# jinggqu/NextGen-UIA

Hardware: AMD Instinct MI355X
Metric: images/sec fwd+bwd BiomedCLIP+Mona bs=256 (higher is better)
Workload: dtype bf16

## Files before the change

include/uia_hip.h:

```cpp
#ifndef UIA_HIP_H
#define UIA_HIP_H
#include <stddef.h>
#include <stdint.h>

#ifdef __cplusplus
extern "C" {
#endif

enum { UIA_F32 = 0, UIA_BF16 = 1 };
enum { UIA_ACT_NONE = 0, UIA_ACT_GELU = 1, UIA_ACT_QUICKGELU = 2, UIA_ACT_RELU = 3 };
enum { UIA_MASK_NONE = 0, UIA_MASK_CAUSAL = 1, UIA_MASK_KEYPAD = 2 };
enum { UIA_MONA_BASELINE = 0, UIA_MONA_NOISE_AWARE = 1, UIA_MONA_FREQ_ENHANCED = 2, UIA_MONA_HYBRID = 3 };

const char* uia_last_error(void);
int uia_version(void);

typedef struct uia_gemm_desc {
    const void* A; int64_t lda;
    const void* W; int64_t ldw;
    int32_t M, N, K;
    float alpha;
    const float* bias;
    int32_t act;
    int32_t dact;
    const void* aux_in; int64_t ldaux_in;
    void* aux_out; int64_t ldaux_out;
    const float* resid; int64_t ldr;
    int32_t resid_mod, resid_row_off;
    const void* residT; int64_t ldrT;
    int32_t out_group;
    void* outT; int64_t ldo;
    float* out32; int64_t ldo32;
    int32_t w_kblocked;
    const void* resid_ln_stats;
    const float* resid_ln_w;
    const float* resid_ln_b;
    int64_t* rowsum_out;
    const int64_t* lnfold_sums;
    const float* lnfold_colsum;
    int32_t lnfold_dim; float lnfold_eps;
    int32_t resid_ln_dim; float resid_ln_eps;
    int64_t a_kb_rows;
    int64_t outT_kb_rows;
    int32_t* ln_flag;
    float ln_flag_limit;
    int32_t drop_where;
    float drop_p;
    uint64_t drop_seed;
    void* a_drop_out;
    float* splitk_ws;
    const void* A2;
    int64_t lda2;
    int32_t K2;
    int32_t a2_group_cols;
    int64_t a2_group_stride;
    const int8_t* resid_lo8;
    int64_t ld_resid_lo;
    int64_t residT_kb_rows;
    int8_t* out_lo8;
    int64_t ld_out_lo;
    int64_t resid_lo_kb_rows;
    int64_t out_lo_kb_rows;
} uia_gemm_desc;
int uia_gemm(void* stream, int dtype, const uia_gemm_desc* d, int tile_cfg );

int uia_wgrad(void* stream, int dtype, int M, int I, int J, const void* A, int64_t lda, const void* B, int64_t ldb,
              float alpha, float* dW, float* dbias_A);
int uia_wgrad_ex(void* stream, int dtype, int M, int I, int J, const void* A, int64_t lda, const void* B, int64_t ldb,
                 float alpha, float* dW, int64_t ldw, int i_valid, int j_valid, float* dbias_A);
int uia_wgrad_drop(void* stream, int dtype, int M, int I, int J, const void* A, int64_t lda, const void* B, int64_t ldb,
                   float alpha, float* dW, int64_t ldw, int i_valid, int j_valid, float drop_p, uint64_t seed, int64_t drop_ld, int drop_col0);
typedef struct uia_wgrad_group_desc {
    int32_t n, M, I, J;
    const void* A[4];
    const void* B[4];
    float* dW[4];
    float* dbias_A[4];
    int64_t lda, ldb, ldw;
    int32_t i_valid, j_valid;
    float alpha, drop_p;
    uint64_t drop_seed[4];
    int64_t drop_ld;
    int32_t drop_col0, reserved;
} uia_wgrad_group_desc;
int uia_wgrad_group(void* stream, int dtype, const uia_wgrad_group_desc* d);

typedef struct uia_attn_desc {
    const void *q, *k, *v; int64_t ld_qkv;
    void* out; int64_t ldo;
    float* lse;
    const int32_t* keylen;
    int32_t B, H, L, dh;
    int32_t mask_kind;
    float scale;
    const void* dout; int64_t lddo;
    void *dq, *dk, *dv; int64_t ld_dqkv;
    const int32_t* cu_seqlens;
    int64_t out_kb_rows;
    int64_t dqkv_kb_rows;
} uia_attn_desc;
int uia_attn_fwd(void* stream, int dtype, const uia_attn_desc* d);
int uia_attn_bwd(void* stream, int dtype, const uia_attn_desc* d);
int uia_attn_bwd_cfg(void* stream, int dtype, const uia_attn_desc* d, int cfg);

int uia_attn_fwd_long(void* stream, int dtype, const uia_attn_desc* d);

int uia_layernorm_fwd(void* stream, int dtype, int M, int D, int64_t ldx, const float* x, const float* gamma, const float* beta,
                      float eps, void* yT, float* y32);
int uia_layernorm_fwd_stats(void* stream, int dtype, int M, int D, int64_t ldx, const float* x, const float* gamma, const float* beta,
                            float eps, void* yT, float* y32, float* stats);
#define UIA_POOL_SLICES 32
int uia_ln_mean_rows(void* stream, int B, int L, int row0, int n, int D, int64_t ldx, const float* x, const float* gamma, const float* beta,
                     float eps, float* ws, float* out, int64_t ldo);
int uia_layernorm_bwd(void* stream, int dtype, int M, int D, int64_t ldx, const void* dy, const float* x, const float* gamma,
                      float eps, const float* dres, float* dx32, void* dxT);
int uia_layernorm_bwd3(void* stream, int dtype, int M, int D, int64_t ldx, const void* dy, const float* x, const void* x_hi, const int8_t* x_lo, int64_t x_kb_rows,
                       const float* gamma, float eps, const float* dres, const void* dres_hi, const int8_t* dres_lo, int64_t dres_kb_rows, float* dx32, void* dxT,
                       int8_t* dx_lo);

typedef struct uia_mona_spatial_desc {
    int32_t variant, B, h, w, bott;
    const void* t;
    void* d;
    const float *conv1_w, *conv1_b, *conv2_w, *conv2_b, *conv3_w, *conv3_b;
    const float *proj_w, *proj_b;
    const float* freq;
    const float *ne1_w, *ne1_b, *ne3_w, *ne3_b;
    float p_drop; uint64_t seed; const uint8_t* keep_mask;
    const void* dd;
    void* dt;
    float *g_conv1_w, *g_conv1_b, *g_conv2_w, *g_conv2_b, *g_conv3_w, *g_conv3_b, *g_proj_w, *g_proj_b, *g_freq,
          *g_ne1_w, *g_ne1_b, *g_ne3_w, *g_ne3_b;
    float* ws;
} uia_mona_spatial_desc;
size_t uia_mona_spatial_workspace_bytes(int B);
int uia_mona_pre_fwd(void* stream, int dtype, int M, int D, const float* x, const float* norm_w, const float* norm_b,
                     const float* gamma, const float* gammax, float eps, void* u);
int uia_mona_pre_fwd_t(void* stream, int dtype, int M, int D, const float* x, const float* norm_w, const float* norm_b, const float* gamma, const float* gammax,
                       float eps, void* u, const void* w1, int64_t ldw1, const float* b1, void* t, int64_t ldt);
int uia_mona_pre_bwd(void* stream, int dtype, int M, int D, const void* du, const float* x, const float* dy,
                     const float* norm_w, const float* norm_b, const float* gamma, const float* gammax, float eps,
                     float* dx32, void* dxT, float* g_gamma, float* g_gammax, float* g_norm_w, float* g_norm_b, float* ws,
                     int64_t dxT_kb_rows);
int uia_mona_pre_bwd_du(void* stream, int dtype, int M, int D, const void* dt, int64_t ldt, const void* w1t, int64_t ldw1, const float* x, const float* dy,
                        const float* norm_w, const float* norm_b, const float* gamma, const float* gammax, float eps,
                        float* dx32, void* dxT, float* g_gamma, float* g_gammax, float* g_norm_w, float* g_norm_b, float* ws, int64_t dxT_kb_rows);
int uia_mona_pre_bwd_du3(void* stream, int dtype, int M, int D, const void* dt, int64_t ldt, const void* w1t, int64_t ldw1, const float* x, const void* dy_hi, const int8_t* dy_lo,
                         const float* norm_w, const float* norm_b, const float* gamma, const float* gammax, float eps, void* dxT, int8_t* dx_lo, float* g_gamma,
                         float* g_gammax, float* g_norm_w, float* g_norm_b, float* ws, int64_t dxT_kb_rows);
size_t uia_mona_pre_bwd_workspace_bytes(int M, int D);
int uia_mona_spatial_fwd(void* stream, int dtype, const uia_mona_spatial_desc* d);
int uia_mona_spatial_bwd(void* stream, int dtype, const uia_mona_spatial_desc* d);

typedef struct uia_mona_fused_desc {
    uia_mona_spatial_desc sp;
    int32_t D; float eps;
    const float* x;
    const float *norm_w, *norm_b, *gamma, *gammax;
    const void* w1; const float* b1;
    const void* w2; const float* b2;
    float* y32;
    void* yT; int64_t yT_kb_rows;
    int64_t* rowsum_out;
    int32_t* ln_flag;
    void* u_out;
    void* t_out;
} uia_mona_fused_desc;
int uia_mona_fused_supported(int dtype, int D, int h, int w, int bott);
int uia_mona_fused_fwd(void* stream, int dtype, const uia_mona_fused_desc* d);

typedef struct uia_lora_rank_desc {
    int32_t M, N, nsrc;
    float alpha;
    const void* Q; int64_t ldq, q_stride;
    const void* W[3]; int64_t ldw;
    void* out; int64_t ldo;
    float drop_p;
    uint64_t seed[3];
} uia_lora_rank_desc;
int uia_lora_rank_update(void* stream, int dtype, const uia_lora_rank_desc* d);

typedef struct uia_ln_lora_desc {
    int32_t M, D, nsrc;
    float eps;
    const float* x; int64_t ldx;
    const float *gamma, *beta;
    void* h;
    const void* A[3]; int64_t lda;
    void* T; int64_t t_stride;
    float drop_p;
    uint64_t seed[3];
} uia_ln_lora_desc;
int uia_ln_lora_down(void* stream, int dtype, const uia_ln_lora_desc* d);

int uia_upsample_bilinear_fwd(void* stream, int B, int C, int h, int w, int H, int W, const float* src, int64_t ld, float* dst);
int uia_upsample_bilinear_bwd(void* stream, int B, int C, int h, int w, int H, int W, const float* ddst, float* dsrc, int64_t ld);
int uia_segment_mean_fwd(void* stream, int B, int n, int C, const float* x, int64_t ld, float* out);
int uia_segment_mean_bwd(void* stream, int B, int n, int C, const float* dout, float* dx, int64_t ld);
size_t uia_dicece_workspace_bytes(int B);
int uia_dicece_fwd_bwd(void* stream, int B, int C, int HW, const float* logits, const float* label, float smooth_nr, float smooth_dr,
                       float* ws, float* loss, float* dlogits);
size_t uia_focal_workspace_bytes(int N, int C);
int uia_focal_fwd_bwd(void* stream, int N, int C, const float* logits, const int64_t* labels, float gamma, float alpha, void* ws, size_t ws_bytes,
                      float* loss, float* dlogits);
size_t uia_binary_cls_stats_workspace_bytes(int N);
int uia_binary_cls_stats(void* stream, int N, const float* p1, const int64_t* labels, const int64_t* perm, void* ws, size_t ws_bytes, double* record);
size_t uia_surface_distances_workspace_bytes(int B, int H, int W);
int uia_surface_distances(void* stream, int B, int H, int W, const float* logits, const float* label, float percentile, void* ws, size_t ws_bytes,
                          double* hd, double* asd);

int uia_cast(void* stream, int dtype, size_t n, const float* src, void* dst, float scale);
int uia_transpose_cast(void* stream, int dtype, int rows, int cols, const float* src, void* dst);

typedef struct uia_pack_desc {
    const float* src;
    void* row;
    void* row_kb;
    void* tr;
    void* tr_kb;
    int32_t rows, cols;
    int32_t rows_pad, cols_pad;
    float scale;
    int32_t reserved_;
} uia_pack_desc;
int uia_pack_weights(void* stream, int dtype, int n, const uia_pack_desc* descs_device, int max_elems);
int uia_im2col(void* stream, int dtype, int B, int C, int H, int W, int P, const float* img, void* out);
int uia_im2col_padded(void* stream, int dtype, int B, int C, int H, int W, int P, const float* img, void* cols, int64_t ldo);
int uia_fill_cls(void* stream, int B, int N, int D, const float* cls, const float* pos0, float* x);
int uia_embed(void* stream, int rows, int L, int D, int vocab, int max_pos, const int64_t* ids, const float* table, const float* pos,
              const float* type0, float* out);
int uia_embed_packed(void* stream, int rows, int D, int vocab, int max_pos, const int64_t* ids, const int64_t* pos_idx, const float* table,
                     const float* pos, const float* type0, float* out);
int uia_embed_bwd(void* stream, int rows, int D, int vocab, const int64_t* ids, const float* dx, float* dtable, int64_t pad_id);
int uia_gather_rows(void* stream, int n, int D, const float* src, const int64_t* idx, float* dst);
int uia_dropout(void* stream, int dtype, size_t n, const void* src, void* dst, float p, uint64_t seed, int accumulate);
int uia_colsum(void* stream, int dtype, int M, int N, const void* A, int64_t lda, float* out);

int uia_layernorm_bwd_affine(void* stream, int dtype, int M, int D, const void* dy, const float* x, const float* gamma, float eps,
                             const float* dres, float* dx32, float* g_gamma, float* g_beta);
int uia_film_fwd(void* stream, int B, int N, int C, const float* x, const float* mul, const float* add, float* y);
int uia_film_bwd(void* stream, int B, int N, int C, const float* dy, const float* x, const float* mul, float* dx, float* dmul, float* dadd);
int uia_im2col3x3(void* stream, int dtype, int B, int h, int w, int C, int ntok, int tok_off, const float* x, void* cols);
int uia_col2im3x3(void* stream, int dtype, int B, int h, int w, int C, int ntok, int tok_off, const void* dcols, float* dx);
int uia_unshuffle(void* stream, int dtype, int B, int h, int w, int k1, int k2, const void* tmp, int64_t ld, float bias, float* out);
int uia_shuffle(void* stream, int dtype, int B, int h, int w, int k1, int k2, const float* dout, void* dtmp, int64_t ld);
int uia_act_bwd(void* stream, int dtype, size_t n, const void* dy, const void* y, int act, void* out);

size_t uia_infonce_workspace_bytes(int B, int E);
int uia_infonce_fwd_bwd(void* stream, int B, int E, const float* img, const float* txt, float inv_temp, float grad_scale,
                        float* loss, float* dimg, float* dtxt, void* workspace, size_t workspace_bytes);

int uia_adamw_clip_step(void* stream, size_t n, float* p, const float* g, float* m, float* v, float lr, float beta1, float beta2,
                        float eps, float weight_decay, float max_norm, int step, float grad_scale, float* ws2);

int uia_grad_accum_guarded(void* stream, size_t n, float* acc, float* mb, const float* loss, float* stats, int32_t* ctl, uint8_t* ok_log, int64_t log_index);
int uia_adamw_clip_step_guarded(void* stream, size_t n, float* p, float* acc, float* m, float* v, float lr, float lr_min, int t_max, float beta1, float beta2,
                                float eps, float weight_decay, float max_norm, float grad_scale, float skip_scale, float* ws8, int32_t* ctl);

enum { UIA_CONV3 = 0, UIA_CONVT_FWD = 1, UIA_CONVT_BWD = 2, UIA_CONV1 = 3 };
#define UIA_WGRAD_MAX_SPLITS 64
#define UIA_WGRAD_MAX_NARROW_SPLITS 512
#define UIA_WGRAD_MAX_DIRECT_SPLITS 1024
int uia_conv_igemm(void* stream, int dtype, int mode, int B, int H, int W, int C1, int C2, const void* x1, const void* x2, int N, int N1,
                   const void* w, const float* bias, void* y1, void* y2);
int uia_conv_wgrad_splits(int mode, int B, int H, int W, int C1, int C2, int N);
int uia_conv_igemm_form(int mode, int C1, int C2, int N, int N1);
int uia_conv_wgrad_form(int mode, int C1, int C2, int N);
int uia_conv_wgrad(void* stream, int dtype, int mode, int B, int H, int W, int C1, int C2, const void* x1, const void* x2, int N, const void* dy,
                   float* ws, float* dw);
#define UIA_BN_SLICES 256
int uia_bn_fwd(void* stream, int dtype, int training, int64_t M, int C, const void* y, const float* gamma, const float* beta, float* running_mean,
               float* running_var, int64_t* num_batches_tracked, float momentum, float eps, float* ws, float* mean, float* invstd, float* scale,
               float* shift, int relu, void* out);
int uia_bn_relu_bwd(void* stream, int dtype, int64_t M, int C, const void* y, const void* dout, const float* scale, const float* shift,
                    const float* mean, const float* invstd, const float* gamma, float* ws, float* dgamma, float* dbeta, void* dy);
int uia_colsum_ordered(void* stream, int dtype, int64_t M, int C, const void* y, float* ws, float* out);
int uia_bn_act_fwd(void* stream, int dtype, int training, int64_t M, int C, const void* y, const float* gamma, const float* beta, float* running_mean,
                   float* running_var, int64_t* num_batches_tracked, float momentum, float eps, float* ws, float* mean, float* invstd, float* scale,
                   float* shift, float slope, void* out, float drop_p, uint64_t seed, const uint8_t* keep_mask);
int uia_bn_act_bwd(void* stream, int dtype, int64_t M, int C, const void* y, const void* dout, const float* scale, const float* shift,
                   const float* mean, const float* invstd, const float* gamma, float* ws, float* dgamma, float* dbeta, void* dy, float slope,
                   float drop_p, uint64_t seed, const uint8_t* keep_mask);
int uia_maxpool2_fwd(void* stream, int dtype, int B, int H, int W, int C, const void* x, void* y);
int uia_maxpool2_bwd(void* stream, int dtype, int B, int H, int W, int C, const void* x, const void* dy, void* dx);
int uia_upsample_ac(void* stream, int dtype, int backward, int B, int H, int W, int C, int f, const void* in, void* out);
int uia_resize_aa(void* stream, int dtype, int backward, int B, int C, int Hi, int Wi, int Ho, int Wo, const void* x, float* tmp, float* out,
                  const float* dout, void* dx);

int uia_conv_strided(void* stream, int dtype, int dgrad, int B, int H, int W, int C, int k, int s, const void* x, int N, const void* w, void* y);
int uia_conv_strided_wgrad_splits(int B, int H, int W, int C, int k, int s, int N);
int uia_conv_strided_form(int dgrad, int C, int N, int k, int s);
int uia_conv_strided_wgrad_form(int C, int N, int k, int s);
int uia_conv_strided_wgrad(void* stream, int dtype, int B, int H, int W, int C, int k, int s, const void* x, int N, const void* dy, float* ws,
                           float* dw);
int uia_maxpool3s2_fwd(void* stream, int dtype, int B, int H, int W, int C, const void* x, void* y);
int uia_maxpool3s2_bwd(void* stream, int dtype, int B, int H, int W, int C, const void* x, const void* dy, void* dx);
int uia_bn_add_relu_fwd(void* stream, int dtype, int training, int64_t M, int C, const void* y, const void* r, const float* gamma, const float* beta,
                        float* running_mean, float* running_var, int64_t* num_batches_tracked, float momentum, float eps, float* ws, float* mean,
                        float* invstd, float* scale, float* shift, void* out);
int uia_bn_add_relu_bwd(void* stream, int dtype, int64_t M, int C, const void* y, const void* out, const void* dout, const float* mean,
                        const float* invstd, const float* gamma, float* ws, float* dgamma, float* dbeta, void* dy, void* dr);
int uia_avgpool_fwd(void* stream, int dtype, int B, int H, int W, int C, const void* x, float* pooled);
int uia_avgpool_bwd(void* stream, int dtype, int B, int H, int W, int C, const float* dout, void* dx);
int uia_nchw_to_nhwc(void* stream, int dtype, int B, int Cin, int H, int W, int Cout, int rep, const float* x, void* out);
int uia_add2(void* stream, int dtype, int64_t n, const void* a, const void* b, void* out);

int uia_comm_unique_id_bytes(void);
int uia_comm_get_unique_id(void* out, int bytes);
int uia_comm_init(int rank, int world, const void* unique_id, int bytes);
int uia_comm_world(void);
int uia_comm_initialised(void);
int uia_allreduce_sum(void* stream, int dtype, void* buf, size_t n);
int uia_allgather(void* stream, int dtype, const void* send, void* recv, size_t n_per_rank);
int uia_comm_destroy(void);

#ifdef __cplusplus
}
// ... 3 lines not shown
```

nextgen-uia_amd/csrc/capi.cpp:

```cpp
#include "uia_kernels.h"

void uia_set_error(const char* fmt, ...);
#define NEED(ptr, name) do { if (!(ptr)) { uia_set_error("%s: null descriptor", name); return -1; } } while (0)

extern "C" {

int uia_version(void) { return 100; }

int uia_gemm(void* stream, int dtype, const uia_gemm_desc* d, int tile_cfg) {
    NEED(d, "uia_gemm");
    return uia_gemm_launch((hipStream_t)stream, dtype, *d, tile_cfg);
}
int uia_lora_rank_update(void* stream, int dtype, const uia_lora_rank_desc* d) {
    NEED(d, "uia_lora_rank_update");
    return uia_lora_rank_update_launch((hipStream_t)stream, dtype, *d);
}
int uia_ln_lora_down(void* stream, int dtype, const uia_ln_lora_desc* d) {
    NEED(d, "uia_ln_lora_down");
    return uia_ln_lora_down_launch((hipStream_t)stream, dtype, *d);
}
int uia_wgrad(void* stream, int dtype, int M, int I, int J, const void* A, int64_t lda, const void* B, int64_t ldb, float alpha, float* dW, float* dbias_A) {
    return uia_wgrad_launch((hipStream_t)stream, dtype, M, I, J, A, lda, B, ldb, alpha, dW, dbias_A);
}
int uia_wgrad_ex(void* stream, int dtype, int M, int I, int J, const void* A, int64_t lda, const void* B, int64_t ldb, float alpha, float* dW, int64_t ldw,
                 int i_valid, int j_valid, float* dbias_A) {
    if (ldw <= 0) { uia_set_error("uia_wgrad_ex: ldw=%lld must be positive", (long long)ldw); return -1; }
    return uia_wgrad_launch((hipStream_t)stream, dtype, M, I, J, A, lda, B, ldb, alpha, dW, dbias_A, ldw, i_valid, j_valid);
}
int uia_wgrad_group(void* stream, int dtype, const uia_wgrad_group_desc* d) {
    if (!d) { uia_set_error("uia_wgrad_group: null descriptor"); return -1; }
    if (d->n < 1 || d->n > 4) { uia_set_error("uia_wgrad_group: n=%d outside 1..4", d->n); return -1; }
    if (d->ldw <= 0) { uia_set_error("uia_wgrad_group: ldw=%lld must be positive", (long long)d->ldw); return -1; }
    float* dW[4];
    float* db[4];
    for (int g = 0; g < 4; ++g) { dW[g] = d->dW[g]; db[g] = d->dbias_A[g]; }
    if (d->drop_p > 0.f) for (int g = 0; g < d->n; ++g) if (db[g]) { uia_set_error("uia_wgrad_group: dbias with dropout on B is not a form of the kernel"); return -1; }
    return uia_wgrad_group_launch((hipStream_t)stream, dtype, d->n, d->M, d->I, d->J, d->A, (long)d->lda, d->B, (long)d->ldb, d->alpha, dW, db, (long)d->ldw, d->i_valid, d->j_valid,
                                  d->drop_p, d->drop_seed, (long)d->drop_ld, d->drop_col0);
}
int uia_wgrad_drop(void* stream, int dtype, int M, int I, int J, const void* A, int64_t lda, const void* B, int64_t ldb, float alpha, float* dW, int64_t ldw,
                   int i_valid, int j_valid, float drop_p, uint64_t seed, int64_t drop_ld, int drop_col0) {
    if (ldw <= 0) { uia_set_error("uia_wgrad_drop: ldw=%lld must be positive", (long long)ldw); return -1; }
    if (!(drop_p > 0.f)) { uia_set_error("uia_wgrad_drop: drop_p=%f must be in (0, 1); uia_wgrad_ex is the form without dropout", (double)drop_p); return -1; }
    return uia_wgrad_launch((hipStream_t)stream, dtype, M, I, J, A, lda, B, ldb, alpha, dW, nullptr, ldw, i_valid, j_valid, drop_p, seed, drop_ld, drop_col0);
}
int uia_attn_fwd(void* stream, int dtype, const uia_attn_desc* d) {
    NEED(d, "uia_attn_fwd");
    return uia_attn_fwd_launch((hipStream_t)stream, dtype, *d);
}
int uia_attn_fwd_long(void* stream, int dtype, const uia_attn_desc* d) {
    NEED(d, "uia_attn_fwd_long");
    return uia_attn_fwd_long_launch((hipStream_t)stream, dtype, *d);
}
int uia_attn_bwd(void* stream, int dtype, const uia_attn_desc* d) {
    NEED(d, "uia_attn_bwd");
    return uia_attn_bwd_launch((hipStream_t)stream, dtype, *d, 0);
}
int uia_attn_bwd_cfg(void* stream, int dtype, const uia_attn_desc* d, int cfg) {
    NEED(d, "uia_attn_bwd_cfg");
    return uia_attn_bwd_launch((hipStream_t)stream, dtype, *d, cfg);
}
int uia_layernorm_fwd(void* stream, int dtype, int M, int D, int64_t ldx, const float* x, const float* gamma, const float* beta, float eps, void* yT, float* y32) {
    return uia_layernorm_fwd_launch((hipStream_t)stream, dtype, M, D, ldx, x, gamma, beta, eps, yT, y32, nullptr);
}
int uia_layernorm_fwd_stats(void* stream, int dtype, int M, int D, int64_t ldx, const float* x, const float* gamma, const float* beta, float eps, void* yT, float* y32,
                            float* stats) {
    return uia_layernorm_fwd_launch((hipStream_t)stream, dtype, M, D, ldx, x, gamma, beta, eps, yT, y32, stats);
}
int uia_layernorm_bwd(void* stream, int dtype, int M, int D, int64_t ldx, const void* dy, const float* x, const float* gamma, float eps, const float* dres, float* dx32, void* dxT) {
    return uia_layernorm_bwd_launch((hipStream_t)stream, dtype, M, D, ldx, dy, x, gamma, eps, dres, dx32, dxT);
}
int uia_layernorm_bwd3(void* stream, int dtype, int M, int D, int64_t ldx, const void* dy, const float* x, const void* x_hi, const int8_t* x_lo, int64_t x_kb_rows,
                       const float* gamma, float eps, const float* dres, const void* dres_hi, const int8_t* dres_lo, int64_t dres_kb_rows, float* dx32, void* dxT,
                       int8_t* dx_lo) {
    return uia_layernorm_bwd3_launch((hipStream_t)stream, dtype, M, D, ldx, dy, x, x_hi, x_lo, (long)x_kb_rows, gamma, eps, dres, dres_hi, dres_lo, (long)dres_kb_rows, dx32, dxT,
                                     dx_lo);
}
int uia_cast(void* stream, int dtype, size_t n, const float* src, void* dst, float scale) { return uia_cast_launch((hipStream_t)stream, dtype, n, src, dst, scale); }
int uia_transpose_cast(void* stream, int dtype, int rows, int cols, const float* src, void* dst) { return uia_transpose_cast_launch((hipStream_t)stream, dtype, rows, cols, src, dst); }
int uia_pack_weights(void* stream, int dtype, int n, const uia_pack_desc* descs_device, int max_elems) { return uia_pack_weights_launch((hipStream_t)stream, dtype, n, descs_device, max_elems); }
int uia_im2col(void* stream, int dtype, int B, int C, int H, int W, int P, const float* img, void* out) { return uia_im2col_launch((hipStream_t)stream, dtype, B, C, H, W, P, img, out); }
int uia_fill_cls(void* stream, int B, int N, int D, const float* cls, const float* pos0, float* x) { return uia_fill_cls_launch((hipStream_t)stream, B, N, D, cls, pos0, x); }
int uia_embed(void* stream, int rows, int L, int D, int vocab, int max_pos, const int64_t* ids, const float* table, const float* pos, const float* type0, float* out) {
    return uia_embed_launch((hipStream_t)stream, rows, L, D, vocab, max_pos, ids, table, pos, type0, out);
}
int uia_gather_rows(void* stream, int n, int D, const float* src, const int64_t* idx, float* dst) { return uia_gather_rows_launch((hipStream_t)stream, n, D, src, idx, dst); }

int uia_mona_pre_fwd(void* stream, int dtype, int M, int D, const float* x, const float* norm_w, const float* norm_b, const float* gamma,
                     const float* gammax, float eps, void* u) {
    return uia_mona_pre_fwd_launch((hipStream_t)stream, dtype, M, D, x, norm_w, norm_b, gamma, gammax, eps, u);
}
int uia_mona_pre_bwd(void* stream, int dtype, int M, int D, const void* du, const float* x, const float* dy, const float* norm_w,
                     const float* norm_b, const float* gamma, const float* gammax, float eps, float* dx32, void* dxT, float* g_gamma,
                     float* g_gammax, float* g_norm_w, float* g_norm_b, float* ws, int64_t dxT_kb_rows) {
    return uia_mona_pre_bwd_launch((hipStream_t)stream, dtype, M, D, du, x, dy, norm_w, norm_b, gamma, gammax, eps, dx32, dxT, g_gamma, g_gammax,
                                   g_norm_w, g_norm_b, ws, (long)dxT_kb_rows);
}
int uia_mona_pre_fwd_t(void* stream, int dtype, int M, int D, const float* x, const float* norm_w, const float* norm_b, const float* gamma, const float* gammax,
                       float eps, void* u, const void* w1, int64_t ldw1, const float* b1, void* t, int64_t ldt) {
    return uia_mona_pre_fwd_t_launch((hipStream_t)stream, dtype, M, D, x, norm_w, norm_b, gamma, gammax, eps, u, w1, (long)ldw1, b1, t, (long)ldt);
}
int uia_mona_pre_bwd_du(void* stream, int dtype, int M, int D, const void* dt, int64_t ldt, const void* w1t, int64_t ldw1, const float* x, const float* dy,
                        const float* norm_w, const float* norm_b, const float* gamma, const float* gammax, float eps, float* dx32, void* dxT, float* g_gamma,
                        float* g_gammax, float* g_norm_w, float* g_norm_b, float* ws, int64_t dxT_kb_rows) {
    if (!dt || !w1t) { uia_set_error("uia_mona_pre_bwd_du: null dt / w1t"); return -1; }
    return uia_mona_pre_bwd_launch((hipStream_t)stream, dtype, M, D, nullptr, x, dy, norm_w, norm_b, gamma, gammax, eps, dx32, dxT, g_gamma, g_gammax,
                                   g_norm_w, g_norm_b, ws, (long)dxT_kb_rows, dt, (long)ldt, w1t, (long)ldw1);
}
int uia_mona_pre_bwd_du3(void* stream, int dtype, int M, int D, const void* dt, int64_t ldt, const void* w1t, int64_t ldw1, const float* x, const void* dy_hi, const int8_t* dy_lo,
                         const float* norm_w, const float* norm_b, const float* gamma, const float* gammax, float eps, void* dxT, int8_t* dx_lo, float* g_gamma,
                         float* g_gammax, float* g_norm_w, float* g_norm_b, float* ws, int64_t dxT_kb_rows) {
    if (!dt || !w1t || !dy_hi || !dy_lo || !dx_lo) { uia_set_error("uia_mona_pre_bwd_du3: null dt / w1t / dy_hi / dy_lo / dx_lo"); return -1; }
    return uia_mona_pre_bwd_launch((hipStream_t)stream, dtype, M, D, nullptr, x, nullptr, norm_w, norm_b, gamma, gammax, eps, nullptr, dxT, g_gamma, g_gammax,
                                   g_norm_w, g_norm_b, ws, (long)dxT_kb_rows, dt, (long)ldt, w1t, (long)ldw1, dy_hi, dy_lo, dx_lo);
}
size_t uia_mona_pre_bwd_workspace_bytes(int M, int D) { return uia_mona_pre_bwd_ws_floats(M, D) * sizeof(float); }
int uia_mona_spatial_fwd(void* stream, int dtype, const uia_mona_spatial_desc* d) {
    NEED(d, "uia_mona_spatial_fwd");
    return uia_mona_spatial_fwd_launch((hipStream_t)stream, dtype, *d);
}
int uia_mona_spatial_bwd(void* stream, int dtype, const uia_mona_spatial_desc* d) {
    NEED(d, "uia_mona_spatial_bwd");
    return uia_mona_spatial_bwd_launch((hipStream_t)stream, dtype, *d);
}
int uia_mona_fused_fwd(void* stream, int dtype, const uia_mona_fused_desc* d) {
    NEED(d, "uia_mona_fused_fwd");
    return uia_mona_fused_fwd_launch((hipStream_t)stream, dtype, *d);
}

size_t uia_infonce_workspace_bytes(int B, int E) { return uia_infonce_workspace_floats(B, E) * sizeof(float); }
int uia_infonce_fwd_bwd(void* stream, int B, int E, const float* img, const float* txt, float inv_temp, float grad_scale, float* loss,
                        float* dimg, float* dtxt, void* workspace, size_t workspace_bytes) {
    return uia_infonce_launch((hipStream_t)stream, B, E, img, txt, inv_temp, grad_scale, loss, dimg, dtxt, (float*)workspace, workspace_bytes / sizeof(float));
}
int uia_adamw_clip_step(void* stream, size_t n, float* p, const float* g, float* m, float* v, float lr, float beta1, float beta2, float eps,
                        float weight_decay, float max_norm, int step, float grad_scale, float* ws2) {
    return uia_adamw_clip_launch((hipStream_t)stream, n, p, g, m, v, lr, beta1, beta2, eps, weight_decay, max_norm, step, grad_scale, ws2);
}
int uia_grad_accum_guarded(void* stream, size_t n, float* acc, float* mb, const float* loss, float* stats, int32_t* ctl, uint8_t* ok_log, int64_t log_index) {
    return uia_grad_accum_guarded_launch((hipStream_t)stream, n, acc, mb, loss, stats, (int*)ctl, ok_log, (long)log_index);
}
int uia_adamw_clip_step_guarded(void* stream, size_t n, float* p, float* acc, float* m, float* v, float lr, float lr_min, int t_max, float beta1, float beta2,
                                float eps, float weight_decay, float max_norm, float grad_scale, float skip_scale, float* ws8, int32_t* ctl) {
    return uia_adamw_clip_guarded_launch((hipStream_t)stream, n, p, acc, m, v, lr, lr_min, t_max, beta1, beta2, eps, weight_decay, max_norm, grad_scale, skip_scale, ws8, (int*)ctl);
}

int uia_dropout(void* stream, int dtype, size_t n, const void* src, void* dst, float p, uint64_t seed, int accumulate) {
    return uia_dropout_launch((hipStream_t)stream, dtype, n, src, dst, p, seed, accumulate);
}
int uia_colsum(void* stream, int dtype, int M, int N, const void* A, int64_t lda, float* out) {
    return uia_colsum_launch((hipStream_t)stream, dtype, M, N, A, lda, out);
}

int uia_layernorm_bwd_affine(void* stream, int dtype, int M, int D, const void* dy, const float* x, const float* gamma, float eps, const float* dres,
                             float* dx32, float* g_gamma, float* g_beta) {
    return uia_layernorm_bwd_affine_launch((hipStream_t)stream, dtype, M, D, dy, x, gamma, eps, dres, dx32, g_gamma, g_beta);
}
int uia_film_fwd(void* stream, int B, int N, int C, const float* x, const float* mul, const float* add, float* y) { return uia_film_fwd_launch((hipStream_t)stream, B, N, C, x, mul, add, y); }
int uia_film_bwd(void* stream, int B, int N, int C, const float* dy, const float* x, const float* mul, float* dx, float* dmul, float* dadd) {
    return uia_film_bwd_launch((hipStream_t)stream, B, N, C, dy, x, mul, dx, dmul, dadd);
// ... 155 lines not shown
```

nextgen-uia_amd/csrc/layernorm.hip:

```cpp
#include "uia_common.h"
#include "uia_kernels.h"

namespace {

constexpr int LN_MAXV = 4;

template <typename T>
__global__ __launch_bounds__(256) void ln_fwd_kernel(int M, int D, long ldx, const float* __restrict__ x, const float* __restrict__ gamma,
                                                      const float* __restrict__ beta, float eps, T* __restrict__ yT, float* __restrict__ y32,
                                                      float* __restrict__ stats) {
    const int row = blockIdx.x * 4 + (threadIdx.x >> 6), lane = threadIdx.x & 63;
    if (row >= M) return;
    const int nv = D >> 2;
    const float* xr = x + (size_t)row * ldx;
    f32x4 v[LN_MAXV];
    float s = 0.f;
#pragma unroll
    for (int k = 0; k < LN_MAXV; ++k) {
        const int c = lane + 64 * k;
        v[k] = c < nv ? load4(xr + 4 * c) : f32x4{0.f, 0.f, 0.f, 0.f};
        s += v[k][0] + v[k][1] + v[k][2] + v[k][3];
    }
    const float mean = wave_sum(s) / D;
    float q = 0.f;
#pragma unroll
    for (int k = 0; k < LN_MAXV; ++k) {
        const int c = lane + 64 * k;
        if (c < nv) {
#pragma unroll
            for (int e = 0; e < 4; ++e) { const float d = v[k][e] - mean; q = fmaf(d, d, q); }
        }
    }
    const float rstd = rsqrtf(wave_sum(q) / D + eps);
    if (stats && lane == 0) *(float2*)(stats + 2 * (size_t)row) = float2{mean, rstd};
#pragma unroll
    for (int k = 0; k < LN_MAXV; ++k) {
        const int c = lane + 64 * k;
        if (c < nv) {
            const f32x4 g = load4(gamma + 4 * c), b = load4(beta + 4 * c);
            f32x4 y;
#pragma unroll
            for (int e = 0; e < 4; ++e) y[e] = fmaf((v[k][e] - mean) * rstd, g[e], b[e]);
            if (yT) store4(yT + (size_t)row * D + 4 * c, y);
            if (y32) store4(y32 + (size_t)row * D + 4 * c, y);
        }
    }
}

template <typename T, bool THREE, int NV>
__global__ __launch_bounds__(256, NV == 4 ? (THREE ? 3 : 5) : 1) void ln_bwd_kernel(int M, int D, long ldx, const T* __restrict__ dy, const float* __restrict__ x,
                                                      const float* __restrict__ gamma, float eps, const float* __restrict__ dres,
                                                      float* __restrict__ dx32, T* __restrict__ dxT,
                                                      const bf16_t* __restrict__ x_hi, const int8_t* __restrict__ x_lo, long x_kb_rows,
                                                      const bf16_t* __restrict__ dres_hi, const int8_t* __restrict__ dres_lo, long dres_kb_rows, int8_t* __restrict__ dx_lo) {
    const int row = blockIdx.x * 4 + (threadIdx.x >> 6), lane = threadIdx.x & 63;
    if (row >= M) return;
    const int nv = D >> 2;
    const float* xr = x + (size_t)row * ldx;
    const T* dyr = dy + (size_t)row * D;
    f32x4 v[NV], g[NV];
    uint2 rhi[THREE ? NV : 1];
    unsigned rlo[THREE ? NV : 1];
    const bool r3 = THREE && dres_lo != nullptr;
    float s = 0.f;
#pragma unroll
    for (int k = 0; k < NV; ++k) {
        const int c = lane + 64 * k;
        v[k] = f32x4{0.f, 0.f, 0.f, 0.f};
        g[k] = f32x4{0.f, 0.f, 0.f, 0.f};
        if constexpr (THREE) { rhi[k] = uint2{0u, 0u}; rlo[k] = 0u; }
        if (c < nv) {
            if (THREE && x_lo) {
                const bf16_t* hp = x_kb_rows ? x_hi + ((size_t)((4 * c) >> 5) * (size_t)x_kb_rows + row) * 32 + ((4 * c) & 31) : x_hi + (size_t)row * D + 4 * c;
                v[k] = three_byte_load4(hp, x_lo + (size_t)row * D + 4 * c);
            } else {
                v[k] = load4(xr + 4 * c);
            }
            const f32x4 d = load4(dyr + 4 * c), w = load4(gamma + 4 * c);
            if constexpr (THREE) {
                if (r3) {
                    rhi[k] = *(const uint2*)(dres_kb_rows ? dres_hi + ((size_t)((4 * c) >> 5) * (size_t)dres_kb_rows + row) * 32 + ((4 * c) & 31) : dres_hi + (size_t)row * D + 4 * c);
                    rlo[k] = *(const unsigned*)(dres_lo + (size_t)row * D + 4 * c);
                }
            }
#pragma unroll
            for (int e = 0; e < 4; ++e) g[k][e] = d[e] * w[e];
        }
        s += v[k][0] + v[k][1] + v[k][2] + v[k][3];
    }
    const float mean = wave_sum(s) / D;
    float q = 0.f;
#pragma unroll
    for (int k = 0; k < NV; ++k) {
        const int c = lane + 64 * k;
#pragma unroll
        for (int e = 0; e < 4; ++e) {
            const float d = c < nv ? v[k][e] - mean : 0.f;
            v[k][e] = d;
            q = fmaf(d, d, q);
        }
    }
    const float rstd = rsqrtf(wave_sum(q) / D + eps);
    float sg = 0.f, sgx = 0.f;
#pragma unroll
    for (int k = 0; k < NV; ++k)
#pragma unroll
        for (int e = 0; e < 4; ++e) {
            v[k][e] *= rstd;
            sg += g[k][e];
            sgx = fmaf(g[k][e], v[k][e], sgx);
        }
    const float mg = wave_sum(sg) / D, mgx = wave_sum(sgx) / D;
#pragma unroll
    for (int k = 0; k < NV; ++k) {
        const int c = lane + 64 * k;
        if (c < nv) {
            f32x4 o = f32x4{0.f, 0.f, 0.f, 0.f};
            if constexpr (THREE) {
                if (r3) o = three_byte_decode4(rhi[k], rlo[k]);
                else if (dres) o = load4(dres + (size_t)row * ldx + 4 * c);
            } else {
                if (dres) o = load4(dres + (size_t)row * ldx + 4 * c);
            }
#pragma unroll
            for (int e = 0; e < 4; ++e) o[e] += rstd * (g[k][e] - mg - v[k][e] * mgx);
            if (dx32) store4(dx32 + (size_t)row * ldx + 4 * c, o);
            if constexpr (sizeof(T) == 2) {
                if (THREE && dx_lo) three_byte_store4((bf16_t*)dxT + (size_t)row * D + 4 * c, dx_lo + (size_t)row * D + 4 * c, o);
                else if (dxT) store4(dxT + (size_t)row * ldx + 4 * c, o);
            } else {
                if (dxT) store4(dxT + (size_t)row * ldx + 4 * c, o);
            }
        }
    }
}

}

int uia_layernorm_fwd_launch(hipStream_t stream, int dtype, int M, int D, long ldx, const float* x, const float* gamma, const float* beta,
                             float eps, void* yT, float* y32, float* stats) {
    UIA_CHECK_ARG(M > 0 && D > 0 && D % 4 == 0 && D <= 1024, "uia_layernorm_fwd: unsupported shape M=%d D=%d", M, D);
    UIA_CHECK_ARG(x && gamma && beta && (yT || y32 || stats), "uia_layernorm_fwd: null tensor");
    UIA_CHECK_ARG(ldx >= D && ldx % 4 == 0, "uia_layernorm_fwd: row stride %ld", ldx);
    UIA_CHECK_ARG(((uintptr_t)x | (uintptr_t)gamma | (uintptr_t)beta | (uintptr_t)yT | (uintptr_t)y32 | (uintptr_t)stats) % 8 == 0, "uia_layernorm_fwd: alignment");
    const dim3 grid((M + 3) / 4), block(256);
    if (dtype == UIA_BF16) hipLaunchKernelGGL(ln_fwd_kernel<bf16_t>, grid, block, 0, stream, M, D, ldx, x, gamma, beta, eps, (bf16_t*)yT, y32, stats);
    else if (dtype == UIA_F32) hipLaunchKernelGGL(ln_fwd_kernel<float>, grid, block, 0, stream, M, D, ldx, x, gamma, beta, eps, (float*)yT, y32, stats);
    else { uia_set_error("uia_layernorm_fwd: bad dtype %d", dtype); return -1; }
    UIA_CHECK_LAUNCH();
    return 0;
}

int uia_layernorm_bwd_launch(hipStream_t stream, int dtype, int M, int D, long ldx, const void* dy, const float* x, const float* gamma, float eps,
                             const float* dres, float* dx32, void* dxT) {
    return uia_layernorm_bwd3_launch(stream, dtype, M, D, ldx, dy, x, nullptr, nullptr, 0, gamma, eps, dres, nullptr, nullptr, 0, dx32, dxT, nullptr);
}

int uia_layernorm_bwd3_launch(hipStream_t stream, int dtype, int M, int D, long ldx, const void* dy, const float* x, const void* x_hi, const int8_t* x_lo,
                              long x_kb_rows, const float* gamma, float eps, const float* dres, const void* dres_hi, const int8_t* dres_lo, long dres_kb_rows,
                              float* dx32, void* dxT, int8_t* dx_lo) {
    UIA_CHECK_ARG(M > 0 && D > 0 && D % 4 == 0 && D <= 1024, "uia_layernorm_bwd: unsupported shape M=%d D=%d", M, D);
    UIA_CHECK_ARG(dy && (x || (x_hi && x_lo)) && gamma && (dx32 || dxT), "uia_layernorm_bwd: null tensor");
    UIA_CHECK_ARG(ldx >= D && ldx % 4 == 0, "uia_layernorm_bwd: row stride %ld", ldx);
    const bool three = x_lo || dres_lo || dx_lo;
    UIA_CHECK_ARG(!three || (dtype == UIA_BF16 && ldx == D), "uia_layernorm_bwd: three-byte tensors need bf16 and compact rows (ldx == D)");
    UIA_CHECK_ARG(!x_lo || (x_hi && !x && (x_kb_rows == 0 || (x_kb_rows >= M && D % 32 == 0)) && ((uintptr_t)x_hi % 8) == 0 && ((uintptr_t)x_lo % 4) == 0),
                  "uia_layernorm_bwd: x as a three-byte tensor needs x_hi + x_lo (and no fp32 x), a K-blocked hi plane of at least M rows and D a multiple of 32");
    UIA_CHECK_ARG(!dres_lo || (dres_hi && !dres && ((uintptr_t)dres_hi % 8) == 0 && ((uintptr_t)dres_lo % 4) == 0), "uia_layernorm_bwd: dres as a three-byte tensor needs dres_hi + dres_lo (and no fp32 dres)");
    UIA_CHECK_ARG(!dx_lo || (dxT && ((uintptr_t)dxT % 8) == 0 && ((uintptr_t)dx_lo % 4) == 0), "uia_layernorm_bwd: dx_lo needs dxT as the hi plane");
    UIA_CHECK_ARG(x_lo || x_kb_rows == 0, "uia_layernorm_bwd: x_kb_rows without a three-byte x");
    UIA_CHECK_ARG(dres_kb_rows == 0 || (dres_lo && dres_kb_rows >= M && D % 32 == 0), "uia_layernorm_bwd: dres_kb_rows needs a three-byte dres, at least M rows per column block and D a multiple of 32");
    const dim3 grid((M + 3) / 4), block(256);
#define UIA_LN_BWD(TT, TH, NVV)                                                                                                              \
    hipLaunchKernelGGL((ln_bwd_kernel<TT, TH, NVV>), grid, block, 0, stream, M, D, ldx, (const TT*)dy, x, gamma, eps, dres, dx32, (TT*)dxT,          \
                       (const bf16_t*)x_hi, x_lo, x_kb_rows, (const bf16_t*)dres_hi, dres_lo, dres_kb_rows, dx_lo)
    const bool narrow = D <= 768;
    if (dtype == UIA_BF16 && three) { if (narrow) UIA_LN_BWD(bf16_t, true, 3); else UIA_LN_BWD(bf16_t, true, 4); }
    else if (dtype == UIA_BF16) { if (narrow) UIA_LN_BWD(bf16_t, false, 3); else UIA_LN_BWD(bf16_t, false, 4); }
    else if (dtype == UIA_F32) { if (narrow) UIA_LN_BWD(float, false, 3); else UIA_LN_BWD(float, false, 4); }
#undef UIA_LN_BWD
    else { uia_set_error("uia_layernorm_bwd: bad dtype %d", dtype); return -1; }
    UIA_CHECK_LAUNCH();
    return 0;
}
```

nextgen-uia_amd/csrc/uia_kernels.h:

```cpp
#pragma once
#include <hip/hip_runtime.h>
#include <stddef.h>
#include <stdint.h>

#include "../../include/uia_hip.h"

typedef uia_gemm_desc UiaGemmParams;
typedef uia_attn_desc UiaAttnParams;

int uia_gemm_launch(hipStream_t stream, int dtype, const UiaGemmParams& p, int cfg);
int uia_attn_fwd_launch(hipStream_t stream, int dtype, const UiaAttnParams& p);
int uia_attn_fwd_long_launch(hipStream_t stream, int dtype, const UiaAttnParams& p);
int uia_attn_bwd_launch(hipStream_t stream, int dtype, const UiaAttnParams& p, int cfg = 0);
int uia_layernorm_fwd_launch(hipStream_t stream, int dtype, int M, int D, long ldx, const float* x, const float* gamma, const float* beta,
                             float eps, void* yT, float* y32, float* stats);
int uia_layernorm_bwd_launch(hipStream_t stream, int dtype, int M, int D, long ldx, const void* dy, const float* x, const float* gamma, float eps,
                             const float* dres, float* dx32, void* dxT);
int uia_layernorm_bwd3_launch(hipStream_t stream, int dtype, int M, int D, long ldx, const void* dy, const float* x, const void* x_hi, const int8_t* x_lo,
                              long x_kb_rows, const float* gamma, float eps, const float* dres, const void* dres_hi, const int8_t* dres_lo, long dres_kb_rows,
                              float* dx32, void* dxT, int8_t* dx_lo);
int uia_lora_rank_update_launch(hipStream_t stream, int dtype, const uia_lora_rank_desc& p);
int uia_ln_lora_down_launch(hipStream_t stream, int dtype, const uia_ln_lora_desc& p);
int uia_cast_launch(hipStream_t stream, int dtype, size_t n, const float* src, void* dst, float scale);
int uia_transpose_cast_launch(hipStream_t stream, int dtype, int rows, int cols, const float* src, void* dst);
int uia_pack_weights_launch(hipStream_t stream, int dtype, int n, const uia_pack_desc* descs_device, int max_elems);
int uia_im2col_launch(hipStream_t stream, int dtype, int B, int C, int H, int W, int P, const float* img, void* out);
int uia_fill_cls_launch(hipStream_t stream, int B, int N, int D, const float* cls, const float* pos0, float* x);
int uia_embed_launch(hipStream_t stream, int rows, int L, int D, int vocab, int max_pos, const int64_t* ids, const float* table, const float* pos, const float* type0, float* out);
int uia_gather_rows_launch(hipStream_t stream, int n, int D, const float* src, const int64_t* idx, float* dst);
int uia_wgrad_group_launch(hipStream_t stream, int dtype, int n, int M, int I, int J, const void* const* A, long lda, const void* const* B, long ldb, float alpha,
                            float* const* dW, float* const* dbias, long ldw, int i_valid, int j_valid, float drop_p, const uint64_t* drop_seed, long drop_ld, int drop_col0);
int uia_wgrad_launch(hipStream_t stream, int dtype, int M, int I, int J, const void* A, long lda, const void* B, long ldb, float alpha, float* dW, float* dbias,
                     long ldw = 0, int i_valid = 0, int j_valid = 0, float drop_p = 0.f, uint64_t drop_seed = 0, long drop_ld = 0, int drop_col0 = 0);
int uia_mona_pre_fwd_launch(hipStream_t stream, int dtype, int M, int D, const float* x, const float* nw, const float* nb, const float* gamma,
                            const float* gammax, float eps, void* u);
int uia_mona_pre_fwd_t_launch(hipStream_t stream, int dtype, int M, int D, const float* x, const float* nw, const float* nb, const float* gamma,
                              const float* gammax, float eps, void* u, const void* w1, long ldw1, const float* b1, void* t, long ldt);
int uia_mona_pre_bwd_launch(hipStream_t stream, int dtype, int M, int D, const void* du, const float* x, const float* dy, const float* nw,
                            const float* nb, const float* gamma, const float* gammax, float eps, float* dx32, void* dxT, float* g_gamma,
                            float* g_gammax, float* g_nw, float* g_nb, float* ws, long dxT_kb_rows, const void* dt = nullptr, long ldt = 0,
                            const void* w1t = nullptr, long ldw1 = 0, const void* dy_hi = nullptr, const int8_t* dy_lo = nullptr, int8_t* dx_lo = nullptr);
size_t uia_mona_pre_bwd_ws_floats(int M, int D);
int uia_mona_spatial_fwd_launch(hipStream_t stream, int dtype, const uia_mona_spatial_desc& p);
int uia_mona_spatial_bwd_launch(hipStream_t stream, int dtype, const uia_mona_spatial_desc& p);
int uia_mona_fused_fwd_launch(hipStream_t stream, int dtype, const uia_mona_fused_desc& q);
size_t uia_infonce_workspace_floats(int B, int E);
int uia_infonce_launch(hipStream_t stream, int B, int E, const float* img, const float* txt, float inv_temp, float grad_scale, float* loss,
                       float* dimg, float* dtxt, float* ws, size_t ws_floats);
int uia_adamw_clip_launch(hipStream_t stream, size_t n, float* p, const float* g, float* m, float* v, float lr, float beta1, float beta2,
                          float eps, float weight_decay, float max_norm, int step, float grad_scale, float* ws);
int uia_grad_accum_guarded_launch(hipStream_t stream, size_t n, float* acc, float* mb, const float* loss, float* stats, int* ctl, unsigned char* ok_log, long log_index);
int uia_adamw_clip_guarded_launch(hipStream_t stream, size_t n, float* p, float* acc, float* m, float* v, float lr, float lr_min, int t_max, float beta1,
                                  float beta2, float eps, float weight_decay, float max_norm, float grad_scale, float skip_scale, float* ws8, int* ctl);
int uia_dropout_launch(hipStream_t stream, int dtype, size_t n, const void* src, void* dst, float p, uint64_t seed, int accumulate);
int uia_colsum_launch(hipStream_t stream, int dtype, int M, int N, const void* A, long lda, float* out);
int uia_attn_small_launch(hipStream_t stream, int dtype, const UiaAttnParams& p, bool bwd);
bool uia_attn_dh16_ok(int dtype, const UiaAttnParams& p);
int uia_attn_dh16_launch(hipStream_t stream, const UiaAttnParams& p, bool bwd);
int uia_layernorm_bwd_affine_launch(hipStream_t stream, int dtype, int M, int D, const void* dy, const float* x, const float* gamma, float eps,
                                    const float* dres, float* dx32, float* g_gamma, float* g_beta);
int uia_film_fwd_launch(hipStream_t stream, int B, int N, int C, const float* x, const float* mul, const float* add, float* y);
int uia_film_bwd_launch(hipStream_t stream, int B, int N, int C, const float* dy, const float* x, const float* mul, float* dx, float* dmul, float* dadd);
int uia_im2col3x3_launch(hipStream_t stream, int dtype, int B, int h, int w, int C, int ntok, int tok_off, const float* x, void* cols);
int uia_col2im3x3_launch(hipStream_t stream, int dtype, int B, int h, int w, int C, int ntok, int tok_off, const void* dcols, float* dx);
int uia_unshuffle_launch(hipStream_t stream, int dtype, int B, int h, int w, int k1, int k2, const void* tmp, long ld, float bias, float* out);
int uia_shuffle_launch(hipStream_t stream, int dtype, int B, int h, int w, int k1, int k2, const float* dout, void* dtmp, long ld);
int uia_act_bwd_launch(hipStream_t stream, int dtype, size_t n, const void* dy, const void* y, int act, void* out);
size_t uia_mona_spatial_ws_floats(int B);
int uia_upsample_bilinear_launch(hipStream_t stream, bool bwd, int B, int C, int h, int w, int H, int W, const float* in, float* out, long ld);
int uia_segment_mean_launch(hipStream_t stream, bool bwd, int B, int n, int C, const float* in, float* out, long ld);
size_t uia_dicece_ws_floats(int B);
int uia_dicece_launch(hipStream_t stream, int B, int C, int HW, const float* logits, const float* label, float nr, float dr, float* ws, float* loss, float* dlogits);
size_t uia_focal_ws_bytes(int N, int C);
int uia_focal_launch(hipStream_t stream, int N, int C, const float* logits, const int64_t* labels, float gamma, float alpha, void* ws, size_t ws_bytes,
                     float* loss, float* dlogits);
size_t uia_binary_cls_stats_ws_bytes(int N);
int uia_binary_cls_stats_launch(hipStream_t stream, int N, const float* p1, const int64_t* labels, const int64_t* perm, void* ws, size_t ws_bytes,
                                double* record);
size_t uia_surface_ws_bytes(int B, int H, int W);
int uia_surface_launch(hipStream_t stream, int B, int H, int W, const float* logits, const float* label, float percentile, void* ws, size_t ws_bytes,
                       double* hd, double* asd);
int uia_im2col_padded_launch(hipStream_t stream, int dtype, int B, int C, int H, int W, int P, const float* img, void* out, long ldo);
int uia_embed_bwd_launch(hipStream_t stream, int rows, int D, int vocab, const int64_t* ids, const float* dx, float* dtable, long pad_id);
int uia_embed_packed_launch(hipStream_t stream, int rows, int D, int vocab, int max_pos, const int64_t* ids, const int64_t* pos_idx, const float* table, const float* pos, const float* type0, float* out);
int uia_ln_mean_rows_launch(hipStream_t stream, int B, int L, int row0, int n, int D, long ldx, const float* x, const float* gamma, const float* beta,
                            float eps, float* ws, float* out, long ldo);
int uia_conv_igemm_launch(hipStream_t stream, int dtype, int mode, int B, int H, int W, int C1, int C2, const void* x1, const void* x2, int N, int N1,
                          const void* w, const float* bias, void* y1, void* y2);
int uia_conv_wgrad_splits(int mode, int B, int H, int W, int C1, int C2, int N);
int uia_conv_wgrad_launch(hipStream_t stream, int dtype, int mode, int B, int H, int W, int C1, int C2, const void* x1, const void* x2, int N,
                          const void* dy, float* ws, float* dw);
int uia_bn_fwd_launch(hipStream_t stream, int dtype, int training, long M, int C, const void* y, const float* gamma, const float* beta,
                      float* run_mean, float* run_var, int64_t* nbt, float momentum, float eps, float* ws, float* mean, float* invstd,
                      float* scale, float* shift, int relu, void* out);
int uia_bn_relu_bwd_launch(hipStream_t stream, int dtype, long M, int C, const void* y, const void* dout, const float* scale, const float* shift,
                           const float* mean, const float* invstd, const float* gamma, float* ws, float* dgamma, float* dbeta, void* dy);
int uia_colsum_ordered_launch(hipStream_t stream, int dtype, long M, int C, const void* y, float* ws, float* out);
int uia_conv_igemm_form(int mode, int C1, int C2, int N, int N1);
int uia_conv_wgrad_form(int mode, int C1, int C2, int N);
int uia_bn_act_fwd_launch(hipStream_t stream, int dtype, int training, long M, int C, const void* y, const float* gamma, const float* beta,
                          float* run_mean, float* run_var, int64_t* nbt, float momentum, float eps, float* ws, float* mean, float* invstd,
                          float* scale, float* shift, float slope, void* out, float drop_p, uint64_t seed, const uint8_t* keep_mask);
int uia_bn_act_bwd_launch(hipStream_t stream, int dtype, long M, int C, const void* y, const void* dout, const float* scale, const float* shift,
// ... 23 lines not shown
```

nextgen-uia_amd/uia_hip/_lib.py:

```python
import ctypes as C
import os
import re

import torch

_HERE = os.path.dirname(os.path.abspath(__file__))
LIB_PATH = os.environ.get("UIA_HIP_LIB") or os.path.join(_HERE, "libuia_hip.so")

F32, BF16 = 0, 1
ACT_NONE, ACT_GELU, ACT_QUICKGELU, ACT_RELU = 0, 1, 2, 3
MASK_NONE, MASK_CAUSAL, MASK_KEYPAD = 0, 1, 2
MONA_VARIANTS = {"baseline": 0, "noise_aware": 1, "freq_enhanced": 2, "hybrid": 3}

vp, i32, i64, f32, sz = C.c_void_p, C.c_int32, C.c_int64, C.c_float, C.c_size_t


class PackDesc(C.Structure):
    _fields_ = [("src", vp), ("row", vp), ("row_kb", vp), ("tr", vp), ("tr_kb", vp), ("rows", i32), ("cols", i32),
                ("rows_pad", i32), ("cols_pad", i32), ("scale", f32), ("reserved_", i32)]


class GemmDesc(C.Structure):
    _fields_ = [("A", vp), ("lda", i64), ("W", vp), ("ldw", i64), ("M", i32), ("N", i32), ("K", i32), ("alpha", f32),
                ("bias", vp), ("act", i32), ("dact", i32), ("aux_in", vp), ("ldaux_in", i64), ("aux_out", vp), ("ldaux_out", i64),
# ... 70 lines not shown
    "uia_conv_wgrad_form": (C.c_int, [C.c_int, C.c_int, C.c_int, C.c_int]),
    "uia_bn_act_fwd": (C.c_int, [vp, C.c_int, C.c_int, i64, C.c_int, vp, vp, vp, vp, vp, vp, f32, f32, vp, vp, vp, vp, vp, f32, vp, f32, C.c_uint64, vp]),
    "uia_bn_act_bwd": (C.c_int, [vp, C.c_int, i64, C.c_int, vp, vp, vp, vp, vp, vp, vp, vp, vp, vp, vp, f32, f32, C.c_uint64, vp]),
    "uia_maxpool2_fwd": (C.c_int, [vp, C.c_int, C.c_int, C.c_int, C.c_int, C.c_int, vp, vp]),
    "uia_maxpool2_bwd": (C.c_int, [vp, C.c_int, C.c_int, C.c_int, C.c_int, C.c_int, vp, vp, vp]),
    "uia_conv_strided": (C.c_int, [vp, C.c_int, C.c_int, C.c_int, C.c_int, C.c_int, C.c_int, C.c_int, C.c_int, vp, C.c_int, vp, vp]),
    "uia_conv_strided_wgrad_splits": (C.c_int, [C.c_int, C.c_int, C.c_int, C.c_int, C.c_int, C.c_int, C.c_int]),
    "uia_conv_strided_form": (C.c_int, [C.c_int, C.c_int, C.c_int, C.c_int, C.c_int]),
    "uia_conv_strided_wgrad_form": (C.c_int, [C.c_int, C.c_int, C.c_int, C.c_int]),
    "uia_conv_strided_wgrad": (C.c_int, [vp, C.c_int, C.c_int, C.c_int, C.c_int, C.c_int, C.c_int, C.c_int, vp, C.c_int, vp, vp, vp]),
    "uia_maxpool3s2_fwd": (C.c_int, [vp, C.c_int, C.c_int, C.c_int, C.c_int, C.c_int, vp, vp]),
    "uia_maxpool3s2_bwd": (C.c_int, [vp, C.c_int, C.c_int, C.c_int, C.c_int, C.c_int, vp, vp, vp]),
    "uia_bn_add_relu_fwd": (C.c_int, [vp, C.c_int, C.c_int, i64, C.c_int, vp, vp, vp, vp, vp, vp, vp, f32, f32, vp, vp, vp, vp, vp, vp]),
    "uia_bn_add_relu_bwd": (C.c_int, [vp, C.c_int, i64, C.c_int, vp, vp, vp, vp, vp, vp, vp, vp, vp, vp, vp]),
    "uia_avgpool_fwd": (C.c_int, [vp, C.c_int, C.c_int, C.c_int, C.c_int, C.c_int, vp, vp]),
    "uia_avgpool_bwd": (C.c_int, [vp, C.c_int, C.c_int, C.c_int, C.c_int, C.c_int, vp, vp]),
    "uia_nchw_to_nhwc": (C.c_int, [vp, C.c_int, C.c_int, C.c_int, C.c_int, C.c_int, C.c_int, C.c_int, vp, vp]),
    "uia_add2": (C.c_int, [vp, C.c_int, i64, vp, vp, vp]),
    "uia_bn_fwd": (C.c_int, [vp, C.c_int, C.c_int, i64, C.c_int, vp, vp, vp, vp, vp, vp, f32, f32, vp, vp, vp, vp, vp, C.c_int, vp]),
    "uia_bn_relu_bwd": (C.c_int, [vp, C.c_int, i64, C.c_int, vp, vp, vp, vp, vp, vp, vp, vp, vp, vp, vp]),
    "uia_colsum_ordered": (C.c_int, [vp, C.c_int, i64, C.c_int, vp, vp, vp]),
    "uia_upsample_ac": (C.c_int, [vp, C.c_int, C.c_int, C.c_int, C.c_int, C.c_int, C.c_int, C.c_int, vp, vp]),
    "uia_resize_aa": (C.c_int, [vp, C.c_int, C.c_int, C.c_int, C.c_int, C.c_int, C.c_int, C.c_int, C.c_int, vp, vp, vp, vp, vp]),
    "uia_layernorm_bwd": (C.c_int, [vp, C.c_int, C.c_int, C.c_int, i64, vp, vp, vp, f32, vp, vp, vp]),
    "uia_ln_lora_down": (C.c_int, [vp, C.c_int, C.POINTER(LnLoraDesc)]),
    "uia_lora_rank_update": (C.c_int, [vp, C.c_int, C.POINTER(LoraRankDesc)]),
    "uia_layernorm_bwd3": (C.c_int, [vp, C.c_int, C.c_int, C.c_int, i64, vp, vp, vp, vp, i64, vp, f32, vp, vp, vp, i64, vp, vp, vp]),
    "uia_mona_pre_fwd": (C.c_int, [vp, C.c_int, C.c_int, C.c_int, vp, vp, vp, vp, vp, f32, vp]),
    "uia_mona_pre_bwd": (C.c_int, [vp, C.c_int, C.c_int, C.c_int, vp, vp, vp, vp, vp, vp, vp, f32, vp, vp, vp, vp, vp, vp, vp, i64]),
    "uia_mona_pre_fwd_t": (C.c_int, [vp, C.c_int, C.c_int, C.c_int, vp, vp, vp, vp, vp, f32, vp, vp, i64, vp, vp, i64]),
    "uia_mona_pre_bwd_du": (C.c_int, [vp, C.c_int, C.c_int, C.c_int, vp, i64, vp, i64, vp, vp, vp, vp, vp, vp, f32, vp, vp, vp, vp, vp, vp, vp, i64]),
    "uia_mona_pre_bwd_du3": (C.c_int, [vp, C.c_int, C.c_int, C.c_int, vp, i64, vp, i64, vp, vp, vp, vp, vp, vp, vp, f32, vp, vp, vp, vp, vp, vp, vp, i64]),
    "uia_mona_pre_bwd_workspace_bytes": (sz, [C.c_int, C.c_int]),
    "uia_mona_spatial_fwd": (C.c_int, [vp, C.c_int, C.POINTER(MonaSpatialDesc)]),
    "uia_mona_spatial_bwd": (C.c_int, [vp, C.c_int, C.POINTER(MonaSpatialDesc)]),
    "uia_mona_spatial_workspace_bytes": (sz, [C.c_int]),
    "uia_mona_fused_supported": (C.c_int, [C.c_int, C.c_int, C.c_int, C.c_int, C.c_int]),
    "uia_mona_fused_fwd": (C.c_int, [vp, C.c_int, C.POINTER(MonaFusedDesc)]),
    "uia_upsample_bilinear_fwd": (C.c_int, [vp, C.c_int, C.c_int, C.c_int, C.c_int, C.c_int, C.c_int, vp, C.c_int64, vp]),
    "uia_upsample_bilinear_bwd": (C.c_int, [vp, C.c_int, C.c_int, C.c_int, C.c_int, C.c_int, C.c_int, vp, vp, C.c_int64]),
    "uia_segment_mean_fwd": (C.c_int, [vp, C.c_int, C.c_int, C.c_int, vp, C.c_int64, vp]),
    "uia_segment_mean_bwd": (C.c_int, [vp, C.c_int, C.c_int, C.c_int, vp, vp, C.c_int64]),
    "uia_dicece_workspace_bytes": (sz, [C.c_int]),
    "uia_dicece_fwd_bwd": (C.c_int, [vp, C.c_int, C.c_int, C.c_int, vp, vp, C.c_float, C.c_float, vp, vp, vp]),
    "uia_focal_workspace_bytes": (sz, [C.c_int, C.c_int]),
    "uia_focal_fwd_bwd": (C.c_int, [vp, C.c_int, C.c_int, vp, vp, f32, f32, vp, sz, vp, vp]),
    "uia_binary_cls_stats_workspace_bytes": (sz, [C.c_int]),
    "uia_binary_cls_stats": (C.c_int, [vp, C.c_int, vp, vp, vp, vp, sz, vp]),
    "uia_surface_distances_workspace_bytes": (sz, [C.c_int, C.c_int, C.c_int]),
    "uia_surface_distances": (C.c_int, [vp, C.c_int, C.c_int, C.c_int, vp, vp, f32, vp, sz, vp, vp]),
    "uia_infonce_workspace_bytes": (sz, [C.c_int, C.c_int]),
    "uia_infonce_fwd_bwd": (C.c_int, [vp, C.c_int, C.c_int, vp, vp, f32, f32, vp, vp, vp, vp, sz]),
    "uia_adamw_clip_step": (C.c_int, [vp, sz, vp, vp, vp, vp, f32, f32, f32, f32, f32, f32, C.c_int, f32, vp]),
    "uia_grad_accum_guarded": (C.c_int, [vp, sz, vp, vp, vp, vp, vp, vp, i64]),
    "uia_adamw_clip_step_guarded": (C.c_int, [vp, sz, vp, vp, vp, vp, f32, f32, C.c_int, f32, f32, f32, f32, f32, f32, f32, vp, vp]),
    "uia_comm_unique_id_bytes": (C.c_int, []),
    "uia_comm_get_unique_id": (C.c_int, [vp, C.c_int]),
    "uia_comm_init": (C.c_int, [C.c_int, C.c_int, vp, C.c_int]),
    "uia_comm_world": (C.c_int, []),
    "uia_comm_initialised": (C.c_int, []),
    "uia_allreduce_sum": (C.c_int, [vp, C.c_int, vp, sz]),
    "uia_allgather": (C.c_int, [vp, C.c_int, vp, vp, sz]),
    "uia_comm_destroy": (C.c_int, []),
    "uia_dropout": (C.c_int, [vp, C.c_int, sz, vp, vp, f32, C.c_uint64, C.c_int]),
    "uia_colsum": (C.c_int, [vp, C.c_int, C.c_int, C.c_int, vp, i64, vp]),
    "uia_layernorm_bwd_affine": (C.c_int, [vp, C.c_int, C.c_int, C.c_int, vp, vp, vp, f32, vp, vp, vp, vp]),
    "uia_film_fwd": (C.c_int, [vp, C.c_int, C.c_int, C.c_int, vp, vp, vp, vp]),
    "uia_film_bwd": (C.c_int, [vp, C.c_int, C.c_int, C.c_int, vp, vp, vp, vp, vp, vp]),
    "uia_im2col3x3": (C.c_int, [vp, C.c_int, C.c_int, C.c_int, C.c_int, C.c_int, C.c_int, C.c_int, vp, vp]),
    "uia_col2im3x3": (C.c_int, [vp, C.c_int, C.c_int, C.c_int, C.c_int, C.c_int, C.c_int, C.c_int, vp, vp]),
    "uia_unshuffle": (C.c_int, [vp, C.c_int, C.c_int, C.c_int, C.c_int, C.c_int, C.c_int, vp, i64, f32, vp]),
    "uia_shuffle": (C.c_int, [vp, C.c_int, C.c_int, C.c_int, C.c_int, C.c_int, C.c_int, vp, vp, i64]),
    "uia_act_bwd": (C.c_int, [vp, C.c_int, sz, vp, vp, C.c_int, vp]),
    "uia_cast": (C.c_int, [vp, C.c_int, sz, vp, vp, f32]),
    "uia_transpose_cast": (C.c_int, [vp, C.c_int, C.c_int, C.c_int, vp, vp]),
    "uia_pack_weights": (C.c_int, [vp, C.c_int, C.c_int, vp, C.c_int]),
    "uia_im2col": (C.c_int, [vp, C.c_int, C.c_int, C.c_int, C.c_int, C.c_int, C.c_int, vp, vp]),
    "uia_im2col_padded": (C.c_int, [vp, C.c_int, C.c_int, C.c_int, C.c_int, C.c_int, C.c_int, vp, vp, C.c_int64]),
    "uia_fill_cls": (C.c_int, [vp, C.c_int, C.c_int, C.c_int, vp, vp, vp]),
    "uia_embed": (C.c_int, [vp, C.c_int, C.c_int, C.c_int, C.c_int, C.c_int, vp, vp, vp, vp, vp]),
    "uia_embed_bwd": (C.c_int, [vp, C.c_int, C.c_int, C.c_int, vp, vp, vp, C.c_int64]),
    "uia_embed_packed": (C.c_int, [vp, C.c_int, C.c_int, C.c_int, C.c_int, vp, vp, vp, vp, vp, vp]),
    "uia_gather_rows": (C.c_int, [vp, C.c_int, C.c_int, vp, vp, vp]),
}

_lib = None
_BLOCKING = ("uia_comm_init", "uia_comm_destroy", "uia_comm_get_unique_id")


class UiaError(RuntimeError):
    pass


def lib():
    global _lib
    if _lib is None:
        if not os.path.exists(LIB_PATH):
            raise UiaError(f"{LIB_PATH} not built: run `make -C nextgen-uia_amd/csrc` (hipcc --offload-arch=gfx950). "
                           "There is no CPU fallback for the uia hot path.")
        release = os.environ.get("UIA_CTYPES_RELEASE_GIL", "0") == "1"
        handle = (C.CDLL if release else C.PyDLL)(LIB_PATH)
        blocking = C.CDLL(LIB_PATH)
        _one_copy_of("librccl")
        _one_copy_of("libamdhip64")
        for name, (res, args) in PROTOTYPES.items():
            fn = getattr(blocking if name in _BLOCKING else handle, name)
            fn.restype, fn.argtypes = res, args
            if name in _BLOCKING:
                setattr(handle, name, fn)
        _lib = handle
    return _lib


def _one_copy_of(stem):
    try:
        pat = re.compile(r"^" + re.escape(stem) + r"\.so(\.\d+)*$")
        paths = {line.split()[-1] for line in open("/proc/self/maps") if pat.match(os.path.basename(line.split()[-1]) if line.split() else "")}
    except OSError:
        return
    real = {os.path.realpath(p) for p in paths}
    if len(real) > 1:
        raise UiaError(f"two copies of {stem} are loaded ({sorted(real)}): import torch before uia_hip so that libuia_hip.so binds to PyTorch's runtime")


def check(rc, what=""):
    if rc != 0:
        raise UiaError(f"{what} failed (rc={rc}): {lib().uia_last_error().decode()}")
```

nextgen-uia_amd/uia_hip/functional.py:

```python
import math
import os
import weakref

import time

import torch

from . import handoff, ops
from ._lib import UiaError
from .handoff import (Resid3, _g3_partner_feeds, fwd3_of, grad3_decode, grad3_of, grad_resid3_enabled, hook_free, linear_chain,
                      publish_fwd3, publish_grad3, publish_rows, publish_t_copy, set_grad_resid3, t_copy_of, take_rows, zero_sums)
from .handoff import clear as clear_t_copies

_STATE = {"dtype": torch.bfloat16, "seed": 0x5EED, "calls": 0, "fwd_resid3": os.environ.get("UIA_FWD_RESID3", "1") != "0"}


def set_compute_dtype(dt):
    assert dt in (torch.bfloat16, torch.float32)
    _STATE["dtype"] = dt


def compute_dtype():
    return _STATE["dtype"]


def set_deferred_text_ln(flag):
    _STATE["text_ln_deferred"] = bool(flag)


def set_block_resid3(flag):
    _STATE["block_resid3"] = bool(flag)


def set_fwd_resid3(flag):
    _STATE["fwd_resid3"] = bool(flag)


def set_text_resid3(flag):
    _STATE["text_resid3"] = bool(flag)


def set_ln_fold(flag):
    _STATE["ln_fold"] = bool(flag)


def set_deterministic(flag):
    _STATE["deterministic"] = bool(flag)
    ops.TAIL_SPLIT_K = not flag


def ln_fold_enabled(dt, rows=None):
    return dt != torch.float32 and _STATE.get("ln_fold", True) and (rows is None or rows > _STATE.get("ln_fold_min_rows", 2048))


class LnFoldRangeError(FloatingPointError):
    """A GEMM that left row sums for a folded LayerNorm saw a non-finite or out-of-range partial sum: the LayerNorm statistics of that
    row — and everything downstream of it — are wrong."""


_FOLD_POLL = {}
_FOLD_REPORTED = {}


POLL_LAG = max(1, int(os.environ.get("UIA_POLL_LAG", "2")))


def reset_ln_flag(device=None):
    dev = torch.device("cuda", torch.cuda.current_device()) if device is None else torch.device(device)
    key = dev.index if dev.index is not None else torch.cuda.current_device()
    _FOLD_POLL.pop(key, None)
    _FOLD_REPORTED.pop(key, None)
    if key in ops._LN_FLAG:
        ops._LN_FLAG[key].zero_()


def poll_ln_flag(device=None, sync=False):
    dev = torch.device("cuda", torch.cuda.current_device()) if device is None else torch.device(device)
    key = dev.index if dev.index is not None else torch.cuda.current_device()
    flag = ops._LN_FLAG.get(key)
    if flag is None:
        return 0
    seen = 0
    pending = _FOLD_POLL.setdefault(key, [])
    while pending and (sync or len(pending) >= POLL_LAG):
        prev = pending.pop(0)
        t0 = time.perf_counter()
        prev[1].synchronize()
        _STATE["gpu_wait_s"] = _STATE.get("gpu_wait_s", 0.0) + time.perf_counter() - t0
        seen |= int(prev[0][0])
    host = torch.empty(1, dtype=torch.int32, pin_memory=True)
    host.copy_(flag, non_blocking=True)
    ev = torch.cuda.Event()
    ev.record()
    if sync:
# ... 234 lines not shown


def _act(M, K, dt, like, n_consumer):
    if ops.kb_ok(M, n_consumer, K, dt):
        return ops.kb_empty(M, K, dt, like.device)
    return torch.empty((M, K), device=like.device, dtype=dt)


def _attn_act(M, K, dt, like, n_consumer):
    return _act(M, K, dt, like, n_consumer) if dt == torch.bfloat16 else torch.empty((M, K), device=like.device, dtype=dt)


def _as_act(buf, M, K, dt, n_consumer):
    if ops.kb_ok(M, n_consumer, K, dt):
        return buf if ops.is_kb(buf) else ops.KBlocked.over(buf.view(M, K))
    return buf.as_rows() if ops.is_kb(buf) else buf


MONA_PARAM_ORDER = ("gamma", "gammax", "project1.weight", "project1.bias", "project2.weight", "project2.bias", "norm.weight", "norm.bias",
                    "adapter_conv.conv1.weight", "adapter_conv.conv1.bias", "adapter_conv.conv2.weight", "adapter_conv.conv2.bias",
                    "adapter_conv.conv3.weight", "adapter_conv.conv3.bias", "adapter_conv.projector.weight", "adapter_conv.projector.bias",
                    "adapter_conv.freq_filter", "adapter_conv.noise_estimator.1.weight", "adapter_conv.noise_estimator.1.bias",
                    "adapter_conv.noise_estimator.3.weight", "adapter_conv.noise_estimator.3.bias")
_SPATIAL_MAP = {"adapter_conv.conv1.weight": "conv1_w", "adapter_conv.conv1.bias": "conv1_b", "adapter_conv.conv2.weight": "conv2_w",
                "adapter_conv.conv2.bias": "conv2_b", "adapter_conv.conv3.weight": "conv3_w", "adapter_conv.conv3.bias": "conv3_b",
                "adapter_conv.projector.weight": "proj_w", "adapter_conv.projector.bias": "proj_b", "adapter_conv.freq_filter": "freq",
                "adapter_conv.noise_estimator.1.weight": "ne1_w", "adapter_conv.noise_estimator.1.bias": "ne1_b",
                "adapter_conv.noise_estimator.3.weight": "ne3_w", "adapter_conv.noise_estimator.3.bias": "ne3_b"}


class MonaFn(torch.autograd.Function):

    @staticmethod
    def forward(ctx, x, variant, hw, p_drop, keep_mask, names, direct, *params):
        P = dict(zip(names, params))
        B, N, D = x.shape
        h, w = hw
        assert N == 1 + h * w, f"Mona expects 1+h*w tokens, got N={N}, hw={hw}"
        dt = compute_dtype()
        x = x.contiguous()
        M = B * N
        bott = P["project1.weight"].shape[0]
        sp = {_SPATIAL_MAP[k]: v.detach().contiguous() for k, v in P.items() if k in _SPATIAL_MAP}
        seed = _next_seed() if (p_drop > 0 and keep_mask is None) else 0
        fold = ln_fold_enabled(dt, M)
        if ops.mona_fused_ok(dt, D, h, w, bott):
            train = any(ctx.needs_input_grad)
            u = _empty((M, D), dt, x) if train else None
            t = _empty((M, bott), dt, x) if train else None
            d = _empty((M, bott), dt, x) if train else None
            w1, w2 = WEIGHTS.get(P["project1.weight"], dt), WEIGHTS.get(P["project2.weight"], dt)
            y = torch.empty_like(x)
            y_t, sums = (_act(M, D, dt, x, 3 * D), zero_sums(M, x.device)) if fold else (None, None)
            ops.mona_fused_fwd(variant, B, h, w, x, P["norm.weight"], P["norm.bias"], P["gamma"], P["gammax"], w1.row, P["project1.bias"], w2.row,
                               P["project2.bias"], sp, y, y_t=y_t, rowsum=sums, u_out=u, t_out=t, d_out=d, p_drop=p_drop, seed=seed, keep_mask=keep_mask)
            if fold:
                publish_rows(y, y_t, sums)
        else:
            u = _empty((M, D), dt, x)
            w1 = WEIGHTS.get(P["project1.weight"], dt)
            t = _empty((M, bott), dt, x)
            if ops.MONA_PRE_FWD_T and x.is_cuda and dt == torch.bfloat16 and D == 768 and bott == 64:
                ops.mona_pre_fwd(x, P["norm.weight"], P["norm.bias"], P["gamma"], P["gammax"], u, proj1=(w1.row if isinstance(w1, ops.PackedW) else w1, P["project1.bias"], t))
            else:
                ops.mona_pre_fwd(x, P["norm.weight"], P["norm.bias"], P["gamma"], P["gammax"], u)
                ops.gemm(u, w1, bias=P["project1.bias"], out_t=t)
            d = _empty((M, bott), dt, x)
            ops.mona_spatial_fwd(variant, B, h, w, t, sp, d, p_drop=p_drop, seed=seed, keep_mask=keep_mask)
            w2 = WEIGHTS.get(P["project2.weight"], dt)
            y = torch.empty_like(x)
            y_t, sums = (_act(M, D, dt, x, 3 * D), zero_sums(M, x.device)) if fold else (None, None)
            three = fold and dt == torch.bfloat16 and _STATE.get("fwd_resid3", True) and handoff.fwd3_consumer_ahead() and M > 2048 and x.is_cuda
            y_lo = torch.empty(M, D, device=x.device, dtype=torch.int8) if three else None
            ops.gemm(d, w2, bias=P["project2.bias"], resid=x.view(M, D), out32=None if three else y.view(M, D), out_t=y_t, out_lo=y_lo, rowsum=sums)
            if three:
                y = publish_fwd3(x.shape, x.device, y_t, y_lo, sums)
            elif fold:
                publish_rows(y, y_t, sums)
        if u is not None:
            ctx.save_for_backward(x, u, t, d, keep_mask if keep_mask is not None else x.new_empty(0), *params)
        ctx.meta = (variant, hw, p_drop, seed, names, keep_mask is not None)
        ctx.direct_params = tuple(params) if direct else None
        ctx.g3_out = dt == torch.bfloat16 and _g3_partner_feeds(x)
        return y

    @staticmethod
    def backward(ctx, dy):
        variant, hw, p_drop, seed, names, has_mask = ctx.meta
        x, u, t, d, keep_mask, *params = ctx.saved_tensors
        keep_mask = keep_mask if has_mask else None
        P = dict(zip(names, params))
        B, N, D = x.shape
        h, w = hw
        M, dt = B * N, u.dtype
        bott = t.shape[1]
        g3 = grad3_of(dy)
        fuse_du = x.is_cuda and ops.mona_pre_bwd_du_ok(M, D, bott, dt)
        if g3 is not None and ops.is_kb(g3.hi):
            dy, g3 = g3.decode().view(B, N, D), None
        if g3 is not None:
            dy_t = g3.hi.view(M, D)
        else:
            dy = dy.contiguous()
            dy_t = t_copy_of(dy, dt).view(M, D)
        direct = ctx.direct_params is not None and all(_is_flat_grad(p) for p in ctx.direct_params)
        G = ({k: p.grad for k, p in zip(names, ctx.direct_params)} if direct
             else {k: torch.zeros_like(v, dtype=torch.float32) for k, v in P.items()})
        w2t = WEIGHTS.get(P["project2.weight"], dt, transpose=True)
        dd = _empty((M, bott), dt, x)
        side = _wgrad_side_stream(x.device) if _STATE.get("wgrad_side_stream", False) else None
        _wgrad_beside(side, lambda: ops.gemm(dy_t, w2t, out_t=dd), dy_t, d, G["project2.weight"], G["project2.bias"])
        sp = {_SPATIAL_MAP[k]: v.detach().contiguous() for k, v in P.items() if k in _SPATIAL_MAP}
        sg = {_SPATIAL_MAP[k]: G[k] for k in P if k in _SPATIAL_MAP}
        dtt = _empty((M, bott), dt, x)
        ops.mona_spatial_bwd(variant, B, h, w, t, sp, dd, dtt, sg, p_drop=p_drop, seed=seed, keep_mask=keep_mask)
        w1t = WEIGHTS.get(P["project1.weight"], dt, transpose=True)
        du = None if fuse_du else _empty((M, D), dt, x)
        _wgrad_beside(side, None if fuse_du else (lambda: ops.gemm(dtt, w1t, out_t=du)), dtt, u, G["project1.weight"], G["project1.bias"])
        need_dx = ctx.needs_input_grad[0]
        dx_t = _act(M, D, dt, x, 4 * D) if (need_dx and dt != torch.float32) else None
        w1t_rows = (dtt, w1t.row if isinstance(w1t, ops.PackedW) else w1t) if fuse_du else None
        if need_dx and g3 is not None and fuse_du and getattr(ctx, "g3_out", False):
            dlo = torch.empty(M, D, device=x.device, dtype=torch.int8)
            ops.mona_pre_bwd(None, x, g3, P["norm.weight"], P["norm.bias"], P["gamma"], P["gammax"], None, dx_t,
                             G["gamma"], G["gammax"], G["norm.weight"], G["norm.bias"], dt_w1t=w1t_rows, dx_lo=dlo)
            dx = publish_grad3(x.shape, x.device, dx_t, dlo)
        else:
            if need_dx and g3 is not None:
                dy = g3.decode().view(B, N, D)
            dx = torch.empty_like(x) if need_dx else None
            ops.mona_pre_bwd(du, x, dy if need_dx else None, P["norm.weight"], P["norm.bias"], P["gamma"], P["gammax"], dx, dx_t,
                             G["gamma"], G["gammax"], G["norm.weight"], G["norm.bias"], dt_w1t=w1t_rows)
            if need_dx:
                publish_t_copy(dx, dx_t)
        grads = tuple(None if direct else (G[k] if ctx.needs_input_grad[7 + i] else None) for i, k in enumerate(names))
        return (dx, None, None, None, None, None, None) + grads


def _wgrad_beside(side, dgrad, a, b, dw, db):
    if side is not None:
        side.wait_stream(torch.cuda.current_stream())
        with torch.cuda.stream(side):
            ops.wgrad(a, b, dw, db)
        a.record_stream(side)
        b.record_stream(side)
    if dgrad is not None:
        dgrad()
    if side is None:
        ops.wgrad(a, b, dw, db)


_WGRAD_SIDE = {}


def _wgrad_side_stream(device):
    key = device.index if device.index is not None else torch.cuda.current_device()
    if key not in _WGRAD_SIDE:
        _WGRAD_SIDE[key] = torch.cuda.Stream(device=device)
    return _WGRAD_SIDE[key]


def set_wgrad_side_stream(flag):
    _STATE["wgrad_side_stream"] = bool(flag)


def join_side_streams():
    cur = torch.cuda.current_stream()
    for st in _WGRAD_SIDE.values():
        cur.wait_stream(st)

# ... 21 lines not shown
        self.heads, self.eps, self.act, self.mask = heads, eps, act, mask
        self.publish_out = publish_out
        self.ln1, self.qkv, self.proj, self.ln2, self.fc1, self.fc2 = ln1, qkv, proj, ln2, fc1, fc2


ATTN_SINGLE_PASS_MAX = 272


class VitBlockFn(torch.autograd.Function):

    @staticmethod
    def forward(ctx, x, spec):
        B, N, D = x.shape
        M, dt = B * N, compute_dtype()
        if N > ATTN_SINGLE_PASS_MAX and (ctx.needs_input_grad[0] or spec.mask is not None):
            raise UiaError(f"vit_block: {N} tokens exceed the {ATTN_SINGLE_PASS_MAX} of the attention backward; sequences this long run forward-only "
                           "(frozen tower under torch.no_grad()), unmasked" if ctx.needs_input_grad[0] else
                           f"vit_block: {N} tokens with a mask: the long attention forward takes no mask")
        x3 = fwd3_of(x)
        like = x3.lo if x3 is not None else x
        if x3 is None:
            x = x.contiguous()
            x2d = x.view(M, D)
        train = ctx.needs_input_grad[0]
        fold = ln_fold_enabled(dt, M)
        if x3 is not None:
            assert fold and dt == torch.bfloat16, "a three-byte forward token reached a block that cannot take it"
            rows = (x3.hi, x3.sums)
        else:
            rows = take_rows(x, dt) if fold else None
        qkv = _empty((M, 3 * D), dt, like)
        if rows is not None:
            wq, cq, bq = WEIGHTS.get_lnfold(spec.qkv[0], spec.qkv[1], spec.ln1[0], spec.ln1[1], dt)
            xin_t, sums0 = rows
            if not ops.is_kb(xin_t):
                xin_t = xin_t.view(M, D)
            ops.gemm(xin_t, wq, bias=bq, out_t=qkv, lnfold=(sums0, cq, D, spec.eps))
            h1 = _act(M, D, dt, like, spec.fc1[0].shape[0]) if x3 is not None else xin_t
        else:
            h1 = _empty((M, D), dt, x)
            ops.layernorm_fwd(x2d, spec.ln1[0], spec.ln1[1], spec.eps, y_t=h1)
            ops.gemm(h1, WEIGHTS.get(spec.qkv[0], dt), bias=spec.qkv[1], out_t=qkv)
        if N > ATTN_SINGLE_PASS_MAX:
            a = _empty((M, D), dt, like)
            ops.attn_fwd_long(qkv[:, :D], qkv[:, D:2 * D], qkv[:, 2 * D:], a, B, spec.heads, N)
            lse = None
        else:
            a = _attn_act(M, D, dt, like, D) if D == 64 * spec.heads else _empty((M, D), dt, like)
            lse = torch.empty(B, spec.heads, N, device=like.device, dtype=torch.float32) if train else None
            ops.attn_fwd(qkv[:, :D], qkv[:, D:2 * D], qkv[:, 2 * D:], a, B, spec.heads, N, lse=lse, mask=spec.mask)
        F = spec.fc1[0].shape[0]
        f = _act(M, F, dt, like, D)
        pre = _empty((M, F), dt, like) if train else None
        r3 = fold and _STATE.get("block_resid3", False) and dt == torch.bfloat16 and M > 2048
        x1 = None if r3 else torch.empty(M, D, device=like.device, dtype=torch.float32)
        lo1 = torch.empty(M, D, device=like.device, dtype=torch.int8) if r3 else None
        if fold:
            sums1 = zero_sums(M, like.device)
            h1 = _as_act(h1, M, D, dt, F) if x3 is None else h1
            resx = dict(resid3=x3.resid3) if x3 is not None else dict(resid=x2d)
            ops.gemm(a, WEIGHTS.get(spec.proj[0], dt), bias=spec.proj[1], out32=x1, out_t=h1, out_lo=lo1, rowsum=sums1, **resx)
            w1, c1, b1 = WEIGHTS.get_lnfold(spec.fc1[0], spec.fc1[1], spec.ln2[0], spec.ln2[1], dt)
            ops.gemm(h1, w1, bias=b1, act=spec.act, aux_out=pre, out_t=f, lnfold=(sums1, c1, D, spec.eps))
        else:
            ops.gemm(a, WEIGHTS.get(spec.proj[0], dt), bias=spec.proj[1], resid=x2d, out32=x1)
            h1 = _as_act(h1, M, D, dt, 0)
            ops.layernorm_fwd(x1, spec.ln2[0], spec.ln2[1], spec.eps, y_t=h1)
            ops.gemm(h1, WEIGHTS.get(spec.fc1[0], dt), bias=spec.fc1[1], act=spec.act, aux_out=pre, out_t=f)
        x2 = torch.empty(B, N, D, device=like.device, dtype=torch.float32)
        res1 = dict(resid3=Resid3(h1, lo1)) if r3 else dict(resid=x1)
        if fold and spec.publish_out:
            sums2 = zero_sums(M, like.device)
            h2 = _act(M, D, dt, like, 3 * D) if r3 else _as_act(h1, M, D, dt, 3 * D)
            ops.gemm(f, WEIGHTS.get(spec.fc2[0], dt), bias=spec.fc2[1], out32=x2.view(M, D), out_t=h2, rowsum=sums2, **res1)
            publish_rows(x2, h2, sums2)
        else:
            ops.gemm(f, WEIGHTS.get(spec.fc2[0], dt), bias=spec.fc2[1], out32=x2.view(M, D), **res1)
        if train:
            saved, ctx.layout = handoff.save_layout(x3.resid3 if x3 is not None else x, qkv, a, lse, Resid3(h1, lo1) if r3 else x1, pre)
            ctx.save_for_backward(*saved)
            ctx.xshape = (B, N, D)
            ctx.spec = spec
            ctx.g3_out = dt == torch.bfloat16 and _g3_partner_feeds(x)
        return x2

    @staticmethod
    def backward(ctx, dx2):
        g3 = grad3_of(dx2)
        xin, qkv, a, lse, x1, pre = handoff.restore_layout(ctx.saved_tensors, ctx.layout)
        x3_in, r3 = isinstance(xin, Resid3), isinstance(x1, Resid3)
        x = xin.lo if x3_in else xin
        spec = ctx.spec
        B, N, D = ctx.xshape
        M, dt = B * N, qkv.dtype
        F = pre.shape[1]
        if g3 is not None:
            dx2_t = g3.hi if ops.is_kb(g3.hi) else g3.hi.view(M, D)
            dres2 = Resid3(dx2_t, g3.lo)
        else:
            dx2 = dx2.contiguous()
            dx2_t = t_copy_of(dx2, dt, allow_kb=True)
            if not ops.is_kb(dx2_t):
                dx2_t = dx2_t.view(M, D)
            dres2 = dx2.view(M, D)
        g3_mode = g3 is not None or getattr(ctx, "g3_out", False)
        dpre = _act(M, F, dt, x, D)
        ops.gemm(dx2_t, WEIGHTS.get(spec.fc2[0], dt, transpose=True), dact=spec.act, aux_in=pre, out_t=dpre)
        dh = _empty((M, D), dt, x)
        ops.gemm(dpre, WEIGHTS.get(spec.fc1[0], dt, transpose=True), out_t=dh)
        del dpre
        if r3 or g3_mode:
            dx1_t = _empty((M, D), dt, x)
            dlo1 = torch.empty(M, D, device=x.device, dtype=torch.int8)
            ops.layernorm_bwd(dh, x1, spec.ln2[0], spec.eps, dres=dres2, dx_t=dx1_t, dx_lo=dlo1)
            dx1 = Resid3(dx1_t, dlo1)
        else:
            dx1 = torch.empty_like(x1)
            dx1_t = _empty((M, D), dt, x) if dt != torch.float32 else dx1
            ops.layernorm_bwd(dh, x1, spec.ln2[0], spec.eps, dres=dres2, dx32=dx1, dx_t=dx1_t if dt != torch.float32 else None)
        da = dh
        ops.gemm(dx1_t, WEIGHTS.get(spec.proj[0], dt, transpose=True), out_t=da)
        dqkv = _attn_act(M, 3 * D, dt, x, D) if D == 64 * spec.heads else _empty((M, 3 * D), dt, x)
        if ops.is_kb(dqkv):
            ops.attn_bwd(qkv[:, :D], qkv[:, D:2 * D], qkv[:, 2 * D:], a, da, lse, dqkv, None, None, B, spec.heads, N, mask=spec.mask)
        else:
            ops.attn_bwd(qkv[:, :D], qkv[:, D:2 * D], qkv[:, 2 * D:], a, da, lse, dqkv[:, :D], dqkv[:, D:2 * D], dqkv[:, 2 * D:], B, spec.heads, N, mask=spec.mask)
        ops.gemm(dqkv, WEIGHTS.get(spec.qkv[0], dt, transpose=True), out_t=da)
        dx_t = _empty((M, D), dt, x) if dt != torch.float32 else None
        xrows = xin if x3_in else x.view(M, D)
        if getattr(ctx, "g3_out", False):
            dlo = torch.empty(M, D, device=x.device, dtype=torch.int8)
            ops.layernorm_bwd(da, xrows, spec.ln1[0], spec.eps, dres=dx1, dx_t=dx_t, dx_lo=dlo)
            return publish_grad3((B, N, D), x.device, dx_t, dlo), None
        dx = torch.empty(B, N, D, device=x.device, dtype=torch.float32)
        ops.layernorm_bwd(da, xrows, spec.ln1[0], spec.eps, dres=dx1, dx32=dx.view(M, D), dx_t=dx_t)
        publish_t_copy(dx, dx_t)
        return dx, None


def vit_block(x, spec):
    return VitBlockFn.apply(x, spec)


class LnResidual:
    __slots__ = ("raw", "stats", "w", "b", "dim", "eps", "hi", "lo")

    def __init__(self, raw, stats, w, b, dim=None, eps=None, hi=None, lo=None):
        self.raw, self.stats, self.w, self.b = raw, stats, w, b
        self.dim, self.eps = dim, eps
        self.hi, self.lo = hi, lo

    def gemm_kw(self):
        if self.lo is not None:
            return dict(resid3=Resid3(self.hi, self.lo), resid_ln=(self.stats, self.w, self.b, self.dim, self.eps))
        if self.stats is None:
            return dict(resid=self.raw)
        if self.dim is None:
            return dict(resid=self.raw, resid_ln=(self.stats, self.w, self.b))
        return dict(resid=self.raw, resid_ln=(self.stats, self.w, self.b, self.dim, self.eps))


def _post_ln(raw, w, b, eps, x_t, stats_buf=None):
    if _STATE.get("text_ln_deferred", True):
        stats = stats_buf if stats_buf is not None else torch.empty(raw.shape[0], 2, device=raw.device, dtype=torch.float32)
        ops.layernorm_fwd(raw, w, b, eps, y_t=x_t, stats=stats)
        return LnResidual(raw, stats, w, b)
    ops.layernorm_fwd(raw, w, b, eps, y_t=x_t, y32=raw)
    return LnResidual(raw, None, w, b)


# ... 37 lines not shown
            res_a = LnResidual(s_a, fold_sums[0], lw_a, lb_a, D, eps)
        w1, c1, b1 = WEIGHTS.get_lnfold(P["intermediate.dense.weight"], P["intermediate.dense.bias"], lw_a, lb_a, dt)
        ops.gemm(s_a_t, w1, bias=b1, act="gelu", out_t=f, lnfold=(fold_sums[0], c1, D, eps))
        if not r3:
            del s_a_t
    else:
        s_a = torch.empty(M, D, device=x_t.device, dtype=torch.float32)
        ops.gemm(a, WEIGHTS.get(P["attention.output.dense.weight"], dt), bias=P["attention.output.dense.bias"], out32=s_a,
                 **(dict(resid_t=x_t) if t_resid else res.gemm_kw()))
        x_t = _as_act(x_t, M, D, dt, 0)
        res_a = _post_ln(s_a, P["attention.output.LayerNorm.weight"], P["attention.output.LayerNorm.bias"], eps, x_t)
        ops.gemm(x_t, WEIGHTS.get(P["intermediate.dense.weight"], dt), bias=P["intermediate.dense.bias"], act="gelu", out_t=f)
    s_o = res.raw if res.raw is not None else torch.empty(M, D, device=x_t.device, dtype=torch.float32)
    if fold and fold_out:
        x_t = _as_act(x_t, M, D, dt, 3 * D)
        if r3:
            lo_o = res.lo if res.lo is not None else torch.empty(M, D, device=x_t.device, dtype=torch.int8)
            ops.gemm(f, WEIGHTS.get(P["output.dense.weight"], dt), bias=P["output.dense.bias"], out_t=x_t, out_lo=lo_o, rowsum=fold_sums[1],
                     **res_a.gemm_kw())
            return LnResidual(None, fold_sums[1], P["output.LayerNorm.weight"], P["output.LayerNorm.bias"], D, eps, hi=x_t, lo=lo_o), x_t
        ops.gemm(f, WEIGHTS.get(P["output.dense.weight"], dt), bias=P["output.dense.bias"], out32=s_o, out_t=x_t, rowsum=fold_sums[1],
                 **res_a.gemm_kw())
        return LnResidual(s_o, fold_sums[1], P["output.LayerNorm.weight"], P["output.LayerNorm.bias"], D, eps), x_t
    ops.gemm(f, WEIGHTS.get(P["output.dense.weight"], dt), bias=P["output.dense.bias"], out32=s_o,
             **(dict(resid_t=x_t) if t_resid else res_a.gemm_kw()))
    stats_buf = res.stats if (res.dim is None and res.stats is not None) else None
    x_t = _as_act(x_t, M, D, dt, 0)
    return _post_ln(s_o, P["output.LayerNorm.weight"], P["output.LayerNorm.bias"], eps, x_t, stats_buf=stats_buf), x_t


_GRAY_W = {}


def gray_conv_weight(conv_w):
    if conv_w.requires_grad:
        raise NotImplementedError("one-channel input through a TRAINABLE patch embedding: widen the batch instead (src.datasets.segmentation.as_model_input)")
    key = id(conv_w)
    hit = _GRAY_W.get(key)
    sig = (conv_w._version, conv_w.data_ptr(), conv_w.dtype, conv_w.device)
    if hit is None or hit[0] != sig or hit[2]() is not conv_w:
        import weakref
        hit = _GRAY_W[key] = (sig, conv_w.detach().float().sum(dim=1, keepdim=True).contiguous(), weakref.ref(conv_w))
    return hit[1]


class PatchEmbedFn(torch.autograd.Function):

    @staticmethod
    def forward(ctx, images, conv_w, conv_b, cls, pos, patch):
        dt = compute_dtype()
        B, C, H, W = images.shape
        G = (H // patch) * (W // patch)
        D = conv_w.shape[0]
        K = C * patch * patch
        gran = 64 if dt == torch.bfloat16 else 32
        Kp = (K + gran - 1) // gran * gran
        cols = _empty((B * G, Kp), dt, images)
        ops.im2col(images.contiguous().float(), cols, patch)
        x = torch.empty(B, G + 1, D, device=images.device, dtype=torch.float32)
        pos2d = pos.detach().reshape(G + 1, D).contiguous()
        ops.gemm(cols, WEIGHTS.get(conv_w, dt, pad_cols_to=Kp), bias=conv_b, resid=pos2d, resid_mod=G, resid_row_off=1, out_group=G, out32=x.view(-1, D))
        ops.fill_cls(x, cls.detach().reshape(D).contiguous(), pos2d[0])
        return x

    @staticmethod
    def backward(ctx, g):
        return None, None, None, None, None, None


class ClsHeadFn(torch.autograd.Function):

    @staticmethod
    def forward(ctx, x, ln_w, ln_b, eps, w, w_is_in_out=False):
        B, N, D = x.shape
        dt = head_dtype()
        x = x.contiguous()
        h = _empty((B, D), dt, x)
        ops.layernorm_fwd(x, ln_w, ln_b, eps, y_t=h, rows=B, ldx=N * D)
        E = w.shape[1] if w_is_in_out else w.shape[0]
        feat = torch.empty(B, E, device=x.device, dtype=torch.float32)
        ops.gemm(h, WEIGHTS.get(w, dt, transpose=w_is_in_out), out32=feat)
        ctx.save_for_backward(x, ln_w)
        ctx.meta = (eps, w, w_is_in_out, dt)
        return feat

    @staticmethod
    def backward(ctx, dfeat):
        x, ln_w = ctx.saved_tensors
        eps, w, w_is_in_out, hdt = ctx.meta
        B, N, D = x.shape
        dt = compute_dtype()
        df = t_copy_of(dfeat.contiguous(), hdt)
        dh = _empty((B, D), hdt, x)
        E = df.shape[1]
        if E % 64:
            Ep = (E + 63) // 64 * 64
            dfp = df.new_zeros(B, Ep)
            dfp[:, :E] = df
            df = dfp
            wt = WEIGHTS.get(w, hdt, transpose=not w_is_in_out, **({"pad_cols_to": Ep} if w_is_in_out else {"pad_rows_to": Ep}))
        else:
            wt = WEIGHTS.get(w, hdt, transpose=not w_is_in_out)
        ops.gemm(df, wt, out_t=dh)
        if hdt != dt:
            dh_t = _empty((B, D), dt, x)
            ops.cast(dh, dh_t)
            dh = dh_t
        dx = torch.zeros_like(x)
        dx_t = torch.zeros(B * N, D, device=x.device, dtype=dt) if dt != torch.float32 else None
        ops.layernorm_bwd(dh, x, ln_w, eps, dx32=dx, dx_t=dx_t, rows=B, ldx=N * D)
        publish_t_copy(dx, dx_t)
        return dx, None, None, None, None, None


class LayerNormFn(torch.autograd.Function):

    @staticmethod
    def forward(ctx, x, w, b, eps):
        D = x.shape[-1]
        x2 = x.contiguous().view(-1, D)
        y = _empty(x2.shape, compute_dtype(), x)
        ops.layernorm_fwd(x2, w, b, eps, y_t=y)
        ctx.save_for_backward(x2, w)
        ctx.meta = (eps, x.shape)
        return y.view(x.shape)

    @staticmethod
    def backward(ctx, dy):
        x2, w = ctx.saved_tensors
        eps, shape = ctx.meta
        dx = torch.empty_like(x2)
        ops.layernorm_bwd(dy.contiguous().view(x2.shape), x2, w, eps, dx32=dx)
        return dx.view(shape), None, None, None


class AttentionFn(torch.autograd.Function):

    @staticmethod
    def forward(ctx, q, k, v, B, H, L, mask):
        kind, keylen = (mask[0], mask[1]) if isinstance(mask, tuple) else (mask, None)
        out = _empty((B * L, H * 64), q.dtype, q)
        need = any(ctx.needs_input_grad[:3])
        lse = torch.empty(B, H, L, device=q.device, dtype=torch.float32) if need else None
        ops.attn_fwd(q, k, v, out, B, H, L, lse=lse, mask=kind, keylen=keylen)
        if need:
            ctx.save_for_backward(q, k, v, out, lse)
            ctx.meta = (B, H, L, kind, keylen)
        return out

    @staticmethod
    def backward(ctx, dout):
        q, k, v, out, lse = ctx.saved_tensors
        B, H, L, kind, keylen = ctx.meta
        D = H * 64
        dqkv = _empty((B * L, 3 * D), q.dtype, q)
        ops.attn_bwd(q, k, v, out, dout.contiguous(), lse, dqkv[:, :D], dqkv[:, D:2 * D], dqkv[:, 2 * D:], B, H, L, mask=kind, keylen=keylen)
        return dqkv[:, :D], dqkv[:, D:2 * D], dqkv[:, 2 * D:], None, None, None, None


class MlpHalfFn(torch.autograd.Function):

    @staticmethod
    def forward(ctx, x1, spec):
        shape = x1.shape
        D = shape[-1]
        x1 = x1.contiguous().view(-1, D)
        M, dt = x1.shape[0], compute_dtype()
        train = ctx.needs_input_grad[0]
        h = _empty((M, D), dt, x1)
        ops.layernorm_fwd(x1, spec.ln2[0], spec.ln2[1], spec.eps, y_t=h)
        F = spec.fc1[0].shape[0]
        f = _empty((M, F), dt, x1)
        pre = _empty((M, F), dt, x1) if train else None
        ops.gemm(h, WEIGHTS.get(spec.fc1[0], dt), bias=spec.fc1[1], act=spec.act, aux_out=pre, out_t=f)
        x2 = torch.empty_like(x1)
        ops.gemm(f, WEIGHTS.get(spec.fc2[0], dt), bias=spec.fc2[1], resid=x1, out32=x2)
        if train:
            ctx.save_for_backward(x1, pre)
            ctx.meta = (spec, shape)
        return x2.view(shape)

    @staticmethod
    def backward(ctx, dx2):
        x1, pre = ctx.saved_tensors
        spec, shape = ctx.meta
        M, D = x1.shape
        dt = pre.dtype
        dx2 = dx2.contiguous().view(M, D)
        dx2_t = t_copy_of(dx2, dt)
        dpre = _empty(pre.shape, dt, x1)
# ... 1004 lines not shown
```

nextgen-uia_amd/uia_hip/handoff.py:

```python
from typing import NamedTuple

import torch

from . import ops

_STATE = {"chain_depth": 0, "fwd3_next_plain": False, "grad_resid3": False}


class Resid3(NamedTuple):
    hi: object
    lo: torch.Tensor

    def decode(self):
        return ops.three_byte_to_float(self.hi, self.lo).contiguous()


class Fwd3(NamedTuple):
    hi: object
    lo: torch.Tensor
    sums: torch.Tensor

    @property
    def resid3(self):
        return Resid3(self.hi, self.lo)


def save_layout(*values):
    tensors, tags = [], []
    for v in values:
        three = isinstance(v, Resid3)
        hi = v.hi if three else v
        kb = ops.is_kb(hi)
        tensors.append(hi.t if kb else hi)
        if three:
            tensors.append(v.lo)
        tags.append(("3" if three else "") + ("kb" if kb else "rows"))
    return tensors, tuple(tags)


def restore_layout(tensors, tags):
    it, out = iter(tensors), []
    for tag in tags:
        hi = next(it)
        if tag.endswith("kb"):
            hi = ops.KBlocked(hi)
        out.append(Resid3(hi, next(it)) if tag[0] == "3" else hi)
    return out


class TokenRegistry:

    def __init__(self, size):
        self.size, self._pools, self._live = size, {}, {}

    def publish(self, shape, device, payload):
        key = (device.type, device.index if device.index is not None else (torch.cuda.current_device() if device.type == "cuda" else 0))
        pool = self._pools.get(key)
        if pool is None:
            pool = self._pools[key] = [torch.full((self.size,), float("nan"), device=device, dtype=torch.float32), 0]
        i = pool[1]
        pool[1] = (i + 1) % self.size
        tok = pool[0][i:i + 1].view((1,) * len(shape)).expand(shape)
        if len(self._live) >= self.size:
            self._live.clear()
        self._live[tok.data_ptr()] = (payload, tok.numel())
        return tok

    def take(self, t):
        if not self._live or t.dim() == 0 or any(st != 0 for st, n in zip(t.stride(), t.shape) if n > 1):
            return None
        payload, numel = self._live.pop(t.data_ptr(), (None, 0))
        return payload if numel == t.numel() else None

    def clear(self):
        self._live.clear()


GRAD3 = TokenRegistry(64)
FWD3 = TokenRegistry(256)
_G3_VIEWS = ("PermuteBackward0", "ViewBackward0", "UnsafeViewBackward0", "TransposeBackward0", "AliasBackward0", "ReshapeAliasBackward0")
_G3_PARTNERS = ("MonaFnBackward", "VitBlockFnBackward")


def publish_grad3(shape, device, hi, lo):
    return GRAD3.publish(shape, device, Resid3(hi, lo))


def grad3_of(g):
    return GRAD3.take(g)


def grad3_decode(hi, lo):
    return Resid3(hi, lo).decode()


def publish_fwd3(shape, device, hi, lo, sums):
    return FWD3.publish(shape, device, Fwd3(hi, lo, sums))


def fwd3_of(x):
    return FWD3.take(x)


def set_grad_resid3(flag):
    _STATE["grad_resid3"] = bool(flag)


def grad_resid3_enabled():
    return _STATE["grad_resid3"]


class linear_chain:

    def __enter__(self):
        _STATE["chain_depth"] += 1
        return self

    def __exit__(self, *exc):
        _STATE["chain_depth"] -= 1
        _STATE["fwd3_next_plain"] = False
        return False

    @staticmethod
    def next_is_plain_block(flag):
        _STATE["fwd3_next_plain"] = bool(flag)


def fwd3_consumer_ahead():
    return _STATE["fwd3_next_plain"] and _STATE["chain_depth"] > 0


def hook_free(*modules):
    import torch.nn.modules.module as _mm
    if _mm._global_forward_hooks or _mm._global_forward_pre_hooks or _mm._global_backward_hooks or getattr(_mm, "_global_backward_pre_hooks", None) \
            or getattr(_mm, "_global_forward_hooks_always_called", None):
        return False
    for mod in modules:
        for m in mod.modules():
            if m._forward_hooks or m._forward_pre_hooks or m._backward_hooks or getattr(m, "_backward_pre_hooks", None):
                return False
    return True


def _g3_partner_feeds(x):
    if not _STATE["grad_resid3"] or _STATE["chain_depth"] <= 0:
        return False
    fn = x.grad_fn
    for _ in range(8):
        if fn is None:
            return False
        name = type(fn).__name__
        if name in _G3_PARTNERS:
            return True
        if name not in _G3_VIEWS or len(fn.next_functions) != 1:
            return False
        fn = fn.next_functions[0][0]
    return False


_T_COPIES = {}


def publish_t_copy(g32, g_t):
    if g_t is not None and g_t.dtype != torch.float32:
        if len(_T_COPIES) >= 256:
            _T_COPIES.clear()
        _T_COPIES[g32.data_ptr()] = (g32, g32._version, g_t)


def t_copy_of(g32, dt, allow_kb=False):
    if dt == torch.float32:
        return g32
    hit = _T_COPIES.pop(g32.data_ptr(), None)
    if hit is not None:
        src, version, g_t = hit
        if (src.shape == g32.shape and src.stride() == g32.stride() and version == g32._version
                and src.untyped_storage().data_ptr() == g32.untyped_storage().data_ptr() and g_t.dtype == dt and (allow_kb or not ops.is_kb(g_t))):
            return g_t
    out = torch.empty(g32.shape, device=g32.device, dtype=dt)
    ops.cast(g32.contiguous(), out)
    return out


_SUMS_ARENA = {}


def zero_sums(M, device, stream=None):
    key = ops.raw_stream() if stream is None else stream
    a = _SUMS_ARENA.get(key)
    if a is None or a[0].shape[1] != M or a[0].device != device or a[1] >= a[0].shape[0]:
        a = [torch.zeros(48, M, 2, device=device, dtype=torch.int64), 0]
        _SUMS_ARENA[key] = a
    a[1] += 1
    return a[0][a[1] - 1]


_ROWS = {}


def publish_rows(x32, x_t, sums, stream=None):
    _ROWS[ops.raw_stream() if stream is None else stream] = (x32, x32._version, x_t, sums)


def take_rows(x32, dt, stream=None):
    hit = _ROWS.pop(ops.raw_stream() if stream is None else stream, None)
    if hit is not None:
        src, version, x_t, sums = hit
        if (src.data_ptr() == x32.data_ptr() and src.numel() == x32.numel() and version == x32._version
                and src.untyped_storage().data_ptr() == x32.untyped_storage().data_ptr() and x32.is_contiguous() and x_t.dtype == dt):
            return x_t, sums
    return None


def clear():
    _T_COPIES.clear()
    _ROWS.clear()
    _SUMS_ARENA.clear()
    GRAD3.clear()
    FWD3.clear()
```

nextgen-uia_amd/uia_hip/ops.py:

```python
import ctypes as C
from typing import NamedTuple

import torch

from . import _lib
from ._lib import AttnDesc, GemmDesc, LnLoraDesc, LoraRankDesc, MonaFusedDesc, MonaSpatialDesc, PackDesc, UiaError, WgradGroupDesc, check, lib

_ACT = {None: 0, "none": 0, "gelu": 1, "quick_gelu": 2, "relu": 3}

GEMM_PROFILE = None


EPI_BIAS, EPI_AUX_OUT, EPI_GELU, EPI_DGELU, EPI_RESID, EPI_RESIDT, EPI_OUT32, EPI_OUTT, EPI_RESID_LN, EPI_GENERIC = 1, 2, 4, 8, 16, 32, 64, 128, 256, -1
EPI_QUICK = 2048
EPI_ROWSUM, EPI_LNFOLD = 512, 1024
EPI_RESID_LO, EPI_OUT_LO = 4096, 8192
_SPECIALISED = {EPI_BIAS | EPI_RESID | EPI_OUT32, EPI_BIAS | EPI_RESIDT | EPI_OUT32, EPI_BIAS | EPI_RESID | EPI_RESID_LN | EPI_OUT32, EPI_OUTT, EPI_BIAS | EPI_OUTT, EPI_BIAS | EPI_GELU | EPI_OUTT, EPI_DGELU | EPI_OUTT,
                EPI_BIAS | EPI_GELU | EPI_AUX_OUT | EPI_OUTT,
                EPI_QUICK | EPI_BIAS | EPI_GELU | EPI_OUTT, EPI_QUICK | EPI_DGELU | EPI_OUTT, EPI_QUICK | EPI_BIAS | EPI_GELU | EPI_AUX_OUT | EPI_OUTT,
                EPI_BIAS | EPI_RESID | EPI_OUT32 | EPI_OUTT | EPI_ROWSUM, EPI_BIAS | EPI_RESID | EPI_RESID_LN | EPI_OUT32 | EPI_OUTT | EPI_ROWSUM,
                EPI_BIAS | EPI_OUTT | EPI_LNFOLD, EPI_BIAS | EPI_GELU | EPI_OUTT | EPI_LNFOLD, EPI_BIAS | EPI_GELU | EPI_AUX_OUT | EPI_OUTT | EPI_LNFOLD,
                EPI_QUICK | EPI_BIAS | EPI_GELU | EPI_OUTT | EPI_LNFOLD, EPI_QUICK | EPI_BIAS | EPI_GELU | EPI_AUX_OUT | EPI_OUTT | EPI_LNFOLD,
                EPI_BIAS | EPI_RESID_LO | EPI_RESID_LN | EPI_OUTT | EPI_OUT_LO | EPI_ROWSUM,
                EPI_BIAS | EPI_RESID | EPI_OUTT | EPI_OUT_LO | EPI_ROWSUM, EPI_BIAS | EPI_RESID_LO | EPI_OUT32,
# ... 718 lines not shown
        if db is not None:
            assert db.dtype == torch.float32 and db.numel() >= w.shape[0]
            d.dbias_A[g] = db.data_ptr()
    if drop is not None:
        p_, seeds = drop
        if ldb != J or (dbias_list is not None and any(x is not None for x in dbias_list)):
            raise UiaError("wgrad_group(drop=...): no bias, and each b must be the whole dropped tensor (contiguous rows)")
        d.drop_p, d.drop_ld, d.drop_col0 = float(p_), J, 0
        for g in range(n):
            d.drop_seed[g] = int(seeds[g]) & 0xFFFFFFFFFFFFFFFF
    check(lib().uia_wgrad_group(_stream(), _code(a0.dtype), C.byref(d)), "uia_wgrad_group")


def _attn_desc(q, k, v, out, lse, B, H, L, mask, keylen, scale, dh=None):
    d = AttnDesc()
    for t in (q, k, v):
        if t.stride(-1) != 1 or t.dtype != q.dtype:
            raise UiaError("attention operands must be unit-stride in the last dim and share a dtype")
    width = q.shape[-1]
    if width % H != 0 or (dh is not None and dh * H != width) or k.shape[-1] != width or v.shape[-1] != width:
        raise UiaError(f"attention: q / k / v are {q.shape[-1]} / {k.shape[-1]} / {v.shape[-1]} columns wide for {H} heads" + (f" of dim {dh}" if dh is not None else ""))
    dh = width // H
    if dh not in (16, 32, 64):
        raise UiaError(f"attention: head dim {dh} unsupported (16, 32 or 64): {width} columns over {H} heads")
    if not is_kb(out) and out.shape[-1] != width:
        raise UiaError(f"attention: out is {out.shape[-1]} columns wide, q / k / v {width}")
    d.q, d.k, d.v, d.ld_qkv = _p(q), _p(k), _p(v), q.stride(-2)
    assert k.stride(-2) == q.stride(-2) == v.stride(-2)
    if is_kb(out):
        rows, cols, d.out_kb_rows = _kb_dims(out, "attention out")
        if rows < B * L or cols != H * dh or dh != 64 or q.dtype != torch.bfloat16:
            raise UiaError(f"attention out (K-blocked {tuple(out.t.shape)}) must hold [{B * L}, {H * dh}] bf16 with head dim 64")
        d.out, d.ldo = _p(out.t), cols
    else:
        d.out, d.ldo = _p(out), out.stride(-2)
    d.lse = _p(lse)
    d.keylen = _p(keylen)
    d.B, d.H, d.L, d.dh = B, H, L, dh
    d.mask_kind = {"none": 0, None: 0, "causal": 1, "keypad": 2}[mask]
    d.scale = scale if scale is not None else dh ** -0.5
    return d


def attn_fwd(q, k, v, out, B, H, L, lse=None, mask=None, keylen=None, scale=None, dh=None, cu_seqlens=None):
    d = _attn_desc(q, k, v, out, lse, B, H, L, mask, keylen, scale, dh)
    if cu_seqlens is not None:
        assert cu_seqlens.dtype == torch.int32 and cu_seqlens.is_contiguous() and cu_seqlens.numel() == B + 1
        d.cu_seqlens = _p(cu_seqlens)
    check(lib().uia_attn_fwd(_stream(), _code(q.dtype), C.byref(d)), "uia_attn_fwd")


def attn_fwd_long(q, k, v, out, B, H, L, lse=None, scale=None):
    if is_kb(out):
        raise UiaError("attn_fwd_long: the output must be a row-major tensor, not K-blocked")
    d = _attn_desc(q, k, v, out, lse, B, H, L, None, None, scale)
    if d.dh != 64:
        raise UiaError(f"attn_fwd_long: head dim {d.dh}, only 64 is supported")
    check(lib().uia_attn_fwd_long(_stream(), _code(q.dtype), C.byref(d)), "uia_attn_fwd_long")


ATTN_BWD_CFG = 0


def attn_bwd(q, k, v, out, dout, lse, dq, dk, dv, B, H, L, mask=None, keylen=None, scale=None, dh=None, cfg=None):
    d = _attn_desc(q, k, v, out, lse, B, H, L, mask, keylen, scale, dh)
    dh = d.dh
    d.dout, d.lddo = _p(dout), dout.stride(-2)
    if is_kb(dq):
        rows, cols, d.dqkv_kb_rows = _kb_dims(dq, "attention dqkv")
        if rows < B * L or cols != 3 * H * dh or dh != 64 or q.dtype != torch.bfloat16 or dk is not None or dv is not None:
            raise UiaError(f"attention dqkv (K-blocked {tuple(dq.t.shape)}) must hold [{B * L}, {3 * H * dh}] bf16 with head dim 64, dk = dv = None")
        part = (H * dh // kb_group(q.dtype)) * d.dqkv_kb_rows * kb_group(q.dtype) * dq.t.element_size()
        d.dq, d.dk, d.dv, d.ld_dqkv = dq.t.data_ptr(), dq.t.data_ptr() + part, dq.t.data_ptr() + 2 * part, cols
    else:
        d.dq, d.dk, d.dv, d.ld_dqkv = _p(dq), _p(dk), _p(dv), dq.stride(-2)
        assert dk.stride(-2) == dq.stride(-2) == dv.stride(-2)
    cfg = ATTN_BWD_CFG if cfg is None else cfg
    if cfg:
        check(lib().uia_attn_bwd_cfg(_stream(), _code(q.dtype), C.byref(d), int(cfg)), "uia_attn_bwd_cfg")
    else:
        check(lib().uia_attn_bwd(_stream(), _code(q.dtype), C.byref(d)), "uia_attn_bwd")


def layernorm_fwd(x, gamma, beta, eps, y_t=None, y32=None, rows=None, ldx=None, stats=None):
    D = gamma.numel()
    rows = x.numel() // D if rows is None else rows
    ldx = D if ldx is None else ldx
    dt = _code(y_t.dtype) if y_t is not None else _lib.F32
    if stats is not None:
        assert stats.dtype == torch.float32 and stats.is_contiguous() and stats.numel() >= 2 * rows
        check(lib().uia_layernorm_fwd_stats(_stream(), dt, rows, D, ldx, _p(x), _p(gamma), _p(beta), eps, _p(y_t), _p(y32), _p(stats)), "uia_layernorm_fwd_stats")
        return
    check(lib().uia_layernorm_fwd(_stream(), dt, rows, D, ldx, _p(x), _p(gamma), _p(beta), eps, _p(y_t), _p(y32)), "uia_layernorm_fwd")


POOL_SLICES = 32


def ln_mean_rows(x, gamma, beta, eps, row0, n, out=None):
    if x.dim() != 3 or x.dtype != torch.float32 or x.stride(-1) != 1 or x.stride(1) != x.shape[2] or x.stride(0) != x.shape[1] * x.shape[2]:
        raise UiaError("ln_mean_rows: x must be a contiguous fp32 [B, L, D] tensor")
    B, L, D = x.shape
    if out is None:
        out = torch.empty(B, D, device=x.device, dtype=torch.float32)
    if out.dtype != torch.float32 or out.stride(-1) != 1 or out.shape[-1] != D or out.shape[0] != B:
        raise UiaError("ln_mean_rows: out must be fp32 [B, D] with unit column stride")
    ws = torch.empty(B * POOL_SLICES * D, device=x.device, dtype=torch.float32)
    check(lib().uia_ln_mean_rows(_stream(), B, L, int(row0), int(n), D, D, _p(x), _p(gamma), _p(beta), float(eps), _p(ws), _p(out), out.stride(0)),
          "uia_ln_mean_rows")
    return out


def layernorm_bwd(dy, x, gamma, eps, dres=None, dx32=None, dx_t=None, rows=None, ldx=None, dx_lo=None):
    D = gamma.numel()
    rows = dy.numel() // D if rows is None else rows
    ldx = D if ldx is None else ldx
    if isinstance(x, tuple) or isinstance(dres, tuple) or dx_lo is not None:
        x_hi, x_lo = x if isinstance(x, tuple) else (None, None)
        r_hi, r_lo = dres if isinstance(dres, tuple) else (None, None)
        x_kb = r_kb = 0
        if is_kb(x_hi):
            kr, kc, x_kb = _kb_dims(x_hi, "layernorm_bwd x hi plane")
            if kr < rows or kc != D:
                raise UiaError(f"layernorm_bwd: K-blocked x hi plane {tuple(x_hi.t.shape)} does not hold [{rows}, {D}]")
            x_hi = x_hi.t
        if is_kb(r_hi):
            kr, kc, r_kb = _kb_dims(r_hi, "layernorm_bwd dres hi plane")
            if kr < rows or kc != D:
                raise UiaError(f"layernorm_bwd: K-blocked dres hi plane {tuple(r_hi.t.shape)} does not hold [{rows}, {D}]")
            r_hi = r_hi.t
        for name, t, dt_ in (("x hi", x_hi, torch.bfloat16), ("x lo", x_lo, torch.int8), ("dres hi", r_hi, torch.bfloat16), ("dres lo", r_lo, torch.int8), ("dx_lo", dx_lo, torch.int8)):
            if t is not None and (t.dtype != dt_ or not t.is_contiguous() or t.numel() < rows * D):
                raise UiaError(f"layernorm_bwd: {name} plane must be a contiguous {dt_} tensor of at least [{rows}, {D}], got {tuple(t.shape)} {t.dtype}")
        check(lib().uia_layernorm_bwd3(_stream(), _code(dy.dtype), rows, D, ldx, _p(dy), None if isinstance(x, tuple) else _p(x), _p(x_hi), _p(x_lo), x_kb, _p(gamma), eps,
                                       None if isinstance(dres, tuple) else _p(dres), _p(r_hi), _p(r_lo), r_kb, _p(dx32), _p(dx_t), _p(dx_lo)), "uia_layernorm_bwd3")
        return
    check(lib().uia_layernorm_bwd(_stream(), _code(dy.dtype), rows, D, ldx, _p(dy), _p(x), _p(gamma), eps, _p(dres), _p(dx32), _p(dx_t)), "uia_layernorm_bwd")


def cast(src, dst, scale=1.0):
    _dense(src, "cast: src", _F32, align=16)
    _dense(dst, "cast: dst", _FT, src.numel(), align="v4")
    check(lib().uia_cast(_stream(), _code(dst.dtype), src.numel(), _p(src), _p(dst), scale), "uia_cast")


def transpose_cast(src, dst):
    _dense(src, "transpose_cast: src", _F32)
    _dense(dst, "transpose_cast: dst", _FT)
    _require(src.dim() == 2 and tuple(dst.shape) == (src.shape[1], src.shape[0]),
             f"transpose_cast: dst shape {tuple(dst.shape)} is not the transpose of src {tuple(src.shape)}")
    check(lib().uia_transpose_cast(_stream(), _code(dst.dtype), src.shape[0], src.shape[1], _p(src), _p(dst)), "uia_transpose_cast")


_PIN_RING, _PIN_SLOTS, _PIN_SLOT = {}, 512, 4096


def pack_table(entries, device):
    arr = (PackDesc * len(entries))()
    max_elems = 0
    for d, ent in zip(arr, entries):
        src, row, row_kb, tr, tr_kb = ent[:5]
        assert src.dtype == torch.float32 and src.dim() == 2 and src.is_contiguous()
        R, Cc = src.shape
        RP, CP, scale = ent[5] if len(ent) > 5 and ent[5] is not None else (R, Cc, 1.0)
        assert RP >= R and CP >= Cc
        d.src, d.rows, d.cols, d.rows_pad, d.cols_pad, d.scale = _p(src), R, Cc, RP, CP, float(scale)
        for name, t in (("row", row), ("row_kb", row_kb), ("tr", tr), ("tr_kb", tr_kb)):
            if isinstance(t, RawDest):
                assert t.view.device == src.device
                setattr(d, name, t.view.data_ptr())
            elif t is not None:
                assert t.is_contiguous() and t.numel() == RP * CP and t.device == src.device
                setattr(d, name, _p(t))
            if t is not None and name.endswith("_kb"):
                g = 64 // (t.view.element_size() if isinstance(t, RawDest) else t.element_size())
                k, kp = (Cc, CP) if name == "row_kb" else (R, RP)
                if -(-k // g) * g > kp:
                    raise UiaError(f"pack_table: {name} needs its K extent {kp} >= {k} rounded up to {g}")
        max_elems = max(max_elems, R * Cc)
    nbytes = C.sizeof(arr)
    dev = torch.device(device)
    if dev.type == "cuda" and nbytes <= _PIN_SLOT:
        key = dev.index if dev.index is not None else torch.cuda.current_device()
        ring = _PIN_RING.get(key)
        if ring is None:
            ring = _PIN_RING[key] = [torch.empty(_PIN_SLOTS, _PIN_SLOT, dtype=torch.uint8).pin_memory(), 0, [None] * _PIN_SLOTS]
        i = ring[1]
        slot = ring[0][i]
        ring[1] = (i + 1) % _PIN_SLOTS
        if ring[2][i] is not None:
            ring[2][i].synchronize()
        C.memmove(slot.data_ptr(), C.addressof(arr), nbytes)
        table = torch.empty(nbytes, dtype=torch.uint8, device=dev)
        table.copy_(slot[:nbytes], non_blocking=True)
        ev = torch.cuda.Event()
        ev.record()
        ring[2][i] = ev
        return table, len(entries), max_elems
    raw = torch.frombuffer(bytearray(bytes(arr)), dtype=torch.uint8).clone()
    return raw.to(device), len(entries), max_elems


def pack_weights(table, n, max_elems, dtype):
    _dense(table, "pack_weights: table", (torch.uint8,), align=8)
    _require(table.is_cuda and table.numel() >= n * C.sizeof(PackDesc), f"pack_weights: a device table of {n} descriptors is required")
    check(lib().uia_pack_weights(_stream(), _code(dtype), n, _p(table), max_elems), "uia_pack_weights")


def im2col(img, out, patch):
    _require(img.dim() == 4 and out.dim() == 2, "im2col: img [B, C, H, W] and out [rows, ld] are required")
    B, Cc, H, W = img.shape
    _require(H % patch == 0 and W % patch == 0, f"im2col: {H}x{W} image is not a whole number of {patch}-pixel patches")
    _dense(img, "im2col: img", _F32, align=16)
    _dense(out, "im2col: out", _FT)
    _require(out.shape[0] == B * (H // patch) * (W // patch) and out.shape[1] >= Cc * patch * patch,
             f"im2col: out shape {tuple(out.shape)}, expected [{B * (H // patch) * (W // patch)}, >= {Cc * patch * patch}]")
    if patch % 4 == 0 and out.shape[1] == Cc * patch * patch and W % 4 == 0:
        check(lib().uia_im2col(_stream(), _code(out.dtype), B, Cc, H, W, patch, _p(img), _p(out)), "uia_im2col")
    else:
        check(lib().uia_im2col_padded(_stream(), _code(out.dtype), B, Cc, H, W, patch, _p(img), _p(out), out.shape[1]), "uia_im2col_padded")


def fill_cls(x, cls, pos0):
    _require(x.dim() == 3, "fill_cls: x [B, N, D] is required")
    B, N, D = x.shape
    _dense(x, "fill_cls: x", _F32)
    _dense(cls, "fill_cls: cls", _F32, D)
    if pos0 is not None:
        _dense(pos0, "fill_cls: pos0", _F32, D)
    check(lib().uia_fill_cls(_stream(), B, N, D, _p(cls), _p(pos0), _p(x)), "uia_fill_cls")


def _embed_tables(what, table, pos, type0, out, rows):
    _require(table.dim() == 2 and pos.dim() == 2 and pos.shape[1] == table.shape[1] and table.shape[1] % 4 == 0,
             f"{what}: table [V, D] and pos [P, D] with D % 4 == 0 are required, got {tuple(table.shape)} and {tuple(pos.shape)}")
    D = table.shape[1]
    _dense(table, f"{what}: table", _F32, align=16)
    _dense(pos, f"{what}: pos", _F32, align=16)
    if type0 is not None:
        _dense(type0, f"{what}: type0", _F32, D, align=16)
    _dense(out, f"{what}: out", _F32, rows * D, align=16)


def embed(ids, table, pos, type0, out):
    rows, L = ids.numel(), ids.shape[-1]
    _dense(ids, "embed: ids", (torch.int64,))
    _embed_tables("embed", table, pos, type0, out, rows)
    check(lib().uia_embed(_stream(), rows, L, table.shape[1], table.shape[0], pos.shape[0], _p(ids), _p(table), _p(pos), _p(type0), _p(out)), "uia_embed")


def embed_packed(ids, pos_idx, table, pos, type0, out):
    _dense(ids, "embed_packed: ids", (torch.int64,))
    _dense(pos_idx, "embed_packed: pos_idx", (torch.int64,), ids.numel())
    _embed_tables("embed_packed", table, pos, type0, out, ids.numel())
    check(lib().uia_embed_packed(_stream(), ids.numel(), out.shape[1], table.shape[0], pos.shape[0], _p(ids), _p(pos_idx), _p(table), _p(pos), _p(type0), _p(out)),
          "uia_embed_packed")


def embed_bwd(ids, dx, dtable, pad_id=-1):
    _dense(ids, "embed_bwd: ids", (torch.int64,))
    _require(dx.dim() >= 1 and dtable.dim() == 2 and dx.shape[-1] == dtable.shape[1], "embed_bwd: dx [.., D] and dtable [V, D] are required")
    _dense(dx, "embed_bwd: dx", _F32, ids.numel() * dtable.shape[1])
    _dense(dtable, "embed_bwd: dtable", _F32)
    check(lib().uia_embed_bwd(_stream(), ids.numel(), dx.shape[-1], dtable.shape[0], _p(ids), _p(dx), _p(dtable), pad_id), "uia_embed_bwd")


def gather_rows(src, idx, dst):
    _dense(idx, "gather_rows: idx", (torch.int64,))
    _require(src.dim() >= 1 and src.shape[-1] % 4 == 0, "gather_rows: src [.., D] with D % 4 == 0 is required")
    _dense(src, "gather_rows: src", _F32, align=16)
    _dense(dst, "gather_rows: dst", _F32, idx.numel() * src.shape[-1], align=16)
    check(lib().uia_gather_rows(_stream(), idx.numel(), src.shape[-1], _p(src), _p(idx), _p(dst)), "uia_gather_rows")


_SPATIAL_KEYS = ("conv1_w", "conv1_b", "conv2_w", "conv2_b", "conv3_w", "conv3_b", "proj_w", "proj_b", "freq", "ne1_w", "ne1_b", "ne3_w", "ne3_b")


def mona_pre_fwd(x, norm_w, norm_b, gamma, gammax, u, eps=1e-5, proj1=None):
    D = gamma.numel()
    if proj1 is not None:
        w1, b1, t = proj1
        M = x.numel() // D
        if u.dtype != torch.bfloat16 or w1.dtype != u.dtype or t.dtype != u.dtype or tuple(w1.shape) != (64, D) or tuple(t.shape) != (M, 64):
            raise UiaError(f"mona_pre_fwd proj1: w1 {tuple(w1.shape)} / t {tuple(t.shape)} must be bf16 [64, {D}] / [{M}, 64]")
        check(lib().uia_mona_pre_fwd_t(_stream(), _code(u.dtype), M, D, _p(x), _p(norm_w), _p(norm_b), _p(gamma), _p(gammax), eps, _p(u), _p(w1), _rowmajor(w1, "w1"),
                                       _p(b1), _p(t), _rowmajor(t, "t")), "uia_mona_pre_fwd_t")
        return
    check(lib().uia_mona_pre_fwd(_stream(), _code(u.dtype), x.numel() // D, D, _p(x), _p(norm_w), _p(norm_b), _p(gamma), _p(gammax), eps, _p(u)), "uia_mona_pre_fwd")


def mona_pre_bwd_du_ok(M, D, bott, dt):
    return MONA_PRE_BWD_DU and dt == torch.bfloat16 and bott == 64 and D % 64 == 0 and 512 < D <= 768


def mona_pre_bwd(du, x, dy, norm_w, norm_b, gamma, gammax, dx32, dx_t, g_gamma, g_gammax, g_norm_w, g_norm_b, eps=1e-5, dt_w1t=None, dx_lo=None):
    D = gamma.numel()
    M = x.numel() // D
    ws = torch.empty(lib().uia_mona_pre_bwd_workspace_bytes(M, D) // 4, device=x.device, dtype=torch.float32)
    kb_rows = 0
    if is_kb(dx_t):
        rows, cols, kb_rows = _kb_dims(dx_t, "mona_pre_bwd dx_t")
        if rows != M or cols != D:
            raise UiaError(f"mona_pre_bwd dx_t (K-blocked {tuple(dx_t.t.shape)}) does not hold [{M}, {D}]")
        dx_t = dx_t.t
    if dt_w1t is not None:
        dtt, w1t = dt_w1t
        if dtt.dtype != torch.bfloat16 or w1t.dtype != torch.bfloat16 or tuple(dtt.shape) != (M, 64) or tuple(w1t.shape) != (D, 64):
            raise UiaError(f"mona_pre_bwd: dt {tuple(dtt.shape)} {dtt.dtype} / W1ᵀ {tuple(w1t.shape)} {w1t.dtype} must be bf16 [{M}, 64] / [{D}, 64]")
        if isinstance(dy, tuple) or dx_lo is not None:
            if not (isinstance(dy, tuple) and dx_lo is not None and dx32 is None and dx_t is not None):
                raise UiaError("mona_pre_bwd: three-byte residual gradients need dy = (hi, lo), dx_lo and dx_t, and no dx32")
            hi, lo = dy
            for name, t_, dt_ in (("dy hi", hi, torch.bfloat16), ("dy lo", lo, torch.int8), ("dx_lo", dx_lo, torch.int8), ("dx_t", dx_t, torch.bfloat16)):
                if t_.dtype != dt_ or not t_.is_contiguous() or t_.numel() < M * D:
                    raise UiaError(f"mona_pre_bwd: {name} plane must be a contiguous {dt_} tensor of at least [{M}, {D}], got {tuple(t_.shape)} {t_.dtype}")
            check(lib().uia_mona_pre_bwd_du3(_stream(), _code(dtt.dtype), M, D, _p(dtt), _rowmajor(dtt, "dt"), _p(w1t), _rowmajor(w1t, "w1t"), _p(x), _p(hi), _p(lo), _p(norm_w),
                                             _p(norm_b), _p(gamma), _p(gammax), eps, _p(dx_t), _p(dx_lo), _p(g_gamma), _p(g_gammax), _p(g_norm_w), _p(g_norm_b), _p(ws),
                                             kb_rows), "uia_mona_pre_bwd_du3")
            return
        check(lib().uia_mona_pre_bwd_du(_stream(), _code(dtt.dtype), M, D, _p(dtt), _rowmajor(dtt, "dt"), _p(w1t), _rowmajor(w1t, "w1t"), _p(x), _p(dy), _p(norm_w),
                                        _p(norm_b), _p(gamma), _p(gammax), eps, _p(dx32), _p(dx_t), _p(g_gamma), _p(g_gammax), _p(g_norm_w), _p(g_norm_b), _p(ws),
                                        kb_rows), "uia_mona_pre_bwd_du")
        return
    check(lib().uia_mona_pre_bwd(_stream(), _code(du.dtype), M, D, _p(du), _p(x), _p(dy), _p(norm_w), _p(norm_b), _p(gamma), _p(gammax),
                                 eps, _p(dx32), _p(dx_t), _p(g_gamma), _p(g_gammax), _p(g_norm_w), _p(g_norm_b), _p(ws), kb_rows), "uia_mona_pre_bwd")


def _spatial_desc(variant, B, h, w, t, params, p_drop, seed, keep_mask):
    d = MonaSpatialDesc()
    d.variant = _lib.MONA_VARIANTS[variant]
    d.B, d.h, d.w, d.bott = B, h, w, t.shape[-1]
    d.t = _p(t)
    for k in _SPATIAL_KEYS:
        v = params.get(k)
        if v is not None:
            assert v.dtype == torch.float32 and v.is_contiguous()
            setattr(d, k, _p(v))
    d.p_drop, d.seed = float(p_drop), int(seed) & 0xFFFFFFFFFFFFFFFF
    if keep_mask is not None:
        assert keep_mask.dtype == torch.uint8 and keep_mask.is_contiguous()
        d.keep_mask = _p(keep_mask)
    return d


MONA_FUSED = False


def mona_fused_ok(dt, D, h, w, bott):
    return MONA_FUSED and dt == torch.bfloat16 and bool(lib().uia_mona_fused_supported(_code(dt), D, h, w, bott))


def mona_fused_fwd(variant, B, h, w, x, norm_w, norm_b, gamma, gammax, w1, b1, w2, b2, params, y32, y_t=None, rowsum=None, u_out=None, t_out=None, d_out=None,
                   p_drop=0.0, seed=0, keep_mask=None, eps=1e-5):
    D = x.shape[-1]
    q = MonaFusedDesc()
    sp = _spatial_desc(variant, B, h, w, w1.new_empty(0, w1.shape[0]) if t_out is None else t_out, params, p_drop, seed, keep_mask)
    sp.t = None
    if d_out is not None:
        sp.d = _p(d_out)
    q.sp = sp
    q.D, q.eps = D, eps
    assert x.dtype == torch.float32 and x.is_contiguous() and y32.dtype == torch.float32 and y32.is_contiguous() and y32.numel() == x.numel()
    assert tuple(w1.shape) == (sp.bott, D) and tuple(w2.shape) == (D, sp.bott) and w1.is_contiguous() and w2.is_contiguous() and w1.dtype == w2.dtype
    q.x, q.norm_w, q.norm_b, q.gamma, q.gammax = _p(x), _p(norm_w), _p(norm_b), _p(gamma), _p(gammax)
    q.w1, q.b1, q.w2, q.b2, q.y32 = _p(w1), _p(b1), _p(w2), _p(b2), _p(y32)
    M = B * (1 + h * w)
    if is_kb(y_t):
        rows, cols, plane = _kb_dims(y_t, "mona_fused y_t")
        if rows < M or cols != D:
            raise UiaError(f"mona_fused y_t (K-blocked {tuple(y_t.t.shape)}) does not hold [{M}, {D}]")
        q.yT, q.yT_kb_rows = _p(y_t.t), plane
    elif y_t is not None:
        assert y_t.dtype == w1.dtype and y_t.is_contiguous() and y_t.numel() == M * D
        q.yT = _p(y_t)
    if rowsum is not None:
        assert rowsum.dtype == torch.int64 and rowsum.is_contiguous() and rowsum.numel() >= 2 * M
        q.rowsum_out, q.ln_flag = _p(rowsum), _p(ln_flag(x.device))
    for name, t, width in (("u_out", u_out, D), ("t_out", t_out, sp.bott)):
        if t is not None:
            assert t.dtype == w1.dtype and t.is_contiguous() and t.numel() == M * width
            setattr(q, name, _p(t))
    check(lib().uia_mona_fused_fwd(_stream(), _code(w1.dtype), C.byref(q)), "uia_mona_fused_fwd")


def mona_spatial_fwd(variant, B, h, w, t, params, d_out, p_drop=0.0, seed=0, keep_mask=None):
    d = _spatial_desc(variant, B, h, w, t, params, p_drop, seed, keep_mask)
    d.d = _p(d_out)
    check(lib().uia_mona_spatial_fwd(_stream(), _code(t.dtype), C.byref(d)), "uia_mona_spatial_fwd")


def mona_spatial_bwd(variant, B, h, w, t, params, dd, dt, grads, p_drop=0.0, seed=0, keep_mask=None):
    d = _spatial_desc(variant, B, h, w, t, params, p_drop, seed, keep_mask)
    d.dd, d.dt = _p(dd), _p(dt)
    ws = torch.empty(lib().uia_mona_spatial_workspace_bytes(B) // 4, device=t.device, dtype=torch.float32)
    d.ws = _p(ws)
    for k in _SPATIAL_KEYS:
        v = grads.get(k)
        if v is not None:
            setattr(d, "g_" + k, _p(v))
    check(lib().uia_mona_spatial_bwd(_stream(), _code(t.dtype), C.byref(d)), "uia_mona_spatial_bwd")


def infonce(img, txt, temperature, grad_scale=1.0, want_grads=True):
    assert img.dtype == torch.float32 and txt.dtype == torch.float32 and img.is_contiguous() and txt.is_contiguous()
    B, E = img.shape
    nbytes = lib().uia_infonce_workspace_bytes(B, E)
    ws = torch.empty(nbytes // 4, device=img.device, dtype=torch.float32)
    loss = torch.empty(1, device=img.device, dtype=torch.float32)
    dimg = torch.empty_like(img) if want_grads else None
    dtxt = torch.empty_like(txt) if want_grads else None
    check(lib().uia_infonce_fwd_bwd(_stream(), B, E, _p(img), _p(txt), 1.0 / temperature, grad_scale, _p(loss), _p(dimg), _p(dtxt), _p(ws), nbytes), "uia_infonce_fwd_bwd")
    return loss, dimg, dtxt


def adamw_clip_step(p, g, m, v, lr, betas, eps, weight_decay, max_norm, step, grad_scale, ws2):
    for t in (p, g, m, v):
        assert t.dtype == torch.float32 and t.is_contiguous() and t.numel() == p.numel()
    check(lib().uia_adamw_clip_step(_stream(), p.numel(), _p(p), _p(g), _p(m), _p(v), lr, betas[0], betas[1], eps, weight_decay, max_norm, step, grad_scale, _p(ws2)), "uia_adamw_clip_step")


def grad_accum_guarded(acc, mb, loss, stats, ctl, ok_log=None, log_index=0):
    n = mb.numel()
    assert acc.dtype == mb.dtype == loss.dtype == stats.dtype == torch.float32 and acc.numel() >= n + 4 and ctl.dtype == torch.int32 and ctl.numel() >= 4
    assert ok_log is None or (ok_log.dtype == torch.uint8 and 0 <= log_index < ok_log.numel())
    check(lib().uia_grad_accum_guarded(_stream(), n, _p(acc), _p(mb), _p(loss), _p(stats), _p(ctl), _p(ok_log), int(log_index)), "uia_grad_accum_guarded")


def adamw_clip_step_guarded(p, acc, m, v, lr, lr_min, t_max, betas, eps, weight_decay, max_norm, grad_scale, skip_scale, ws8, ctl):
    n = p.numel()
    for t in (p, m, v):
        assert t.dtype == torch.float32 and t.is_contiguous() and t.numel() == n
    assert acc.dtype == torch.float32 and acc.numel() >= n + 4 and ws8.numel() >= 8 and ctl.dtype == torch.int32 and ctl.numel() >= 4
    check(lib().uia_adamw_clip_step_guarded(_stream(), n, _p(p), _p(acc), _p(m), _p(v), lr, lr_min, int(t_max), betas[0], betas[1], eps, weight_decay, max_norm,
                                            grad_scale, skip_scale, _p(ws8), _p(ctl)), "uia_adamw_clip_step_guarded")


def comm_unique_id():
    n = lib().uia_comm_unique_id_bytes()
    buf = C.create_string_buffer(n)
    check(lib().uia_comm_get_unique_id(buf, n), "uia_comm_get_unique_id")
    return bytes(buf.raw)


def comm_init(rank, world, uid):
    check(lib().uia_comm_init(rank, world, C.c_char_p(uid), len(uid)), "uia_comm_init")


def comm_world():
    return lib().uia_comm_world()


def comm_world_initialised():
    return bool(lib().uia_comm_initialised())


def allreduce_sum(buf):
    import os
    try:
        check(lib().uia_allreduce_sum(_stream(), _code(buf.dtype), _p(buf), buf.numel()), "uia_allreduce_sum")
    except UiaError as e:
        raise UiaError(f"rank {os.environ.get('RANK', '0')}/{os.environ.get('WORLD_SIZE', '1')}: {e}") from e


def allgather(send, recv):
    assert send.is_contiguous() and recv.is_contiguous() and send.dtype == recv.dtype and recv.numel() == send.numel() * comm_world()
    check(lib().uia_allgather(_stream(), _code(send.dtype), _p(send), _p(recv), send.numel()), "uia_allgather")


def comm_destroy():
    check(lib().uia_comm_destroy(), "uia_comm_destroy")


def dropout(src, dst, p, seed, accumulate=False):
    assert src.dtype == dst.dtype and src.is_contiguous() and dst.is_contiguous() and src.numel() == dst.numel()
    check(lib().uia_dropout(_stream(), _code(src.dtype), src.numel(), _p(src), _p(dst), p, int(seed) & 0xFFFFFFFFFFFFFFFF, int(accumulate)), "uia_dropout")


def ln_lora_down_ok(D, r, dt):
    return LN_LORA_DOWN and dt == torch.bfloat16 and D in (768, 1024) and 0 < r <= 16


def ln_lora_down(x, gamma, beta, eps, h, a_rows, t_all, drop_p=0.0, seeds=()):
    n, M, w = t_all.shape
    D = gamma.numel()
    if not (t_all.is_contiguous() and w == 64 and len(a_rows) == n and tuple(h.shape) == (M, D) and h.is_contiguous() and x.dtype == torch.float32 and x.shape[-1] == D):
# ... 623 lines not shown
```

Baseline: 6495.

## Exploit CLS-only gradient in last block backward with specialized kernels

Adds a sparse backward path for the case where only the CLS token's output receives gradient, as in image pooling. A CLS-query attention backward kernel computes dq for row 0 and dk/dv for all keys from one query row, a periodic layernorm backward injects the residual gradient only every period-th row, and a Mona CLS backward handles just the CLS rows. Gradients travel as compact per-image rows through a token registry instead of dense [B, L, D] tensors. This skips full attention and adapter backward work for the final block, but adds complexity, extra autograd plumbing and narrower preconditions.

```diff
diff --git a/include/uia_hip.h b/include/uia_hip.h
--- a/include/uia_hip.h
+++ b/include/uia_hip.h
@@ -105,6 +105,8 @@
 
 int uia_attn_fwd_long(void* stream, int dtype, const uia_attn_desc* d);
 
+int uia_attn_bwd_cls(void* stream, int dtype, const uia_attn_desc* d);
+
 int uia_layernorm_fwd(void* stream, int dtype, int M, int D, int64_t ldx, const float* x, const float* gamma, const float* beta,
                       float eps, void* yT, float* y32);
 int uia_layernorm_fwd_stats(void* stream, int dtype, int M, int D, int64_t ldx, const float* x, const float* gamma, const float* beta,
@@ -117,6 +119,8 @@
 int uia_layernorm_bwd3(void* stream, int dtype, int M, int D, int64_t ldx, const void* dy, const float* x, const void* x_hi, const int8_t* x_lo, int64_t x_kb_rows,
                        const float* gamma, float eps, const float* dres, const void* dres_hi, const int8_t* dres_lo, int64_t dres_kb_rows, float* dx32, void* dxT,
                        int8_t* dx_lo);
+int uia_layernorm_bwd_periodic(void* stream, int dtype, int M, int D, const void* dy, const float* x, const void* x_hi, const int8_t* x_lo, int64_t x_kb_rows,
+                               const float* gamma, float eps, const float* dres_rows, int period, float* dx32, void* dxT, int8_t* dx_lo);
 
 typedef struct uia_mona_spatial_desc {
     int32_t variant, B, h, w, bott;
@@ -151,6 +155,8 @@
 size_t uia_mona_pre_bwd_workspace_bytes(int M, int D);
 int uia_mona_spatial_fwd(void* stream, int dtype, const uia_mona_spatial_desc* d);
 int uia_mona_spatial_bwd(void* stream, int dtype, const uia_mona_spatial_desc* d);
+int uia_mona_cls_bwd(void* stream, int dtype, int B, int ntok, const void* dd, const void* t, int64_t ldt, void* dt, float p_drop, uint64_t seed,
+                     const uint8_t* keep_mask);
 
 typedef struct uia_mona_fused_desc {
     uia_mona_spatial_desc sp;
@@ -233,6 +239,7 @@
                      const float* pos, const float* type0, float* out);
 int uia_embed_bwd(void* stream, int rows, int D, int vocab, const int64_t* ids, const float* dx, float* dtable, int64_t pad_id);
 int uia_gather_rows(void* stream, int n, int D, const float* src, const int64_t* idx, float* dst);
+int uia_copy_rows(void* stream, int rows, int64_t row_bytes, const void* src, int64_t src_stride_bytes, void* dst);
 int uia_dropout(void* stream, int dtype, size_t n, const void* src, void* dst, float p, uint64_t seed, int accumulate);
 int uia_colsum(void* stream, int dtype, int M, int N, const void* A, int64_t lda, float* out);
 
diff --git a/nextgen-uia_amd/csrc/capi.cpp b/nextgen-uia_amd/csrc/capi.cpp
--- a/nextgen-uia_amd/csrc/capi.cpp
+++ b/nextgen-uia_amd/csrc/capi.cpp
@@ -76,6 +76,20 @@
     return uia_layernorm_bwd3_launch((hipStream_t)stream, dtype, M, D, ldx, dy, x, x_hi, x_lo, (long)x_kb_rows, gamma, eps, dres, dres_hi, dres_lo, (long)dres_kb_rows, dx32, dxT,
                                      dx_lo);
 }
+int uia_layernorm_bwd_periodic(void* stream, int dtype, int M, int D, const void* dy, const float* x, const void* x_hi, const int8_t* x_lo, int64_t x_kb_rows,
+                               const float* gamma, float eps, const float* dres_rows, int period, float* dx32, void* dxT, int8_t* dx_lo) {
+    return uia_layernorm_bwd_periodic_launch((hipStream_t)stream, dtype, M, D, dy, x, x_hi, x_lo, (long)x_kb_rows, gamma, eps, dres_rows, period, dx32, dxT, dx_lo);
+}
+int uia_attn_bwd_cls(void* stream, int dtype, const uia_attn_desc* d) {
+    NEED(d, "uia_attn_bwd_cls");
+    return uia_attn_bwd_cls_launch((hipStream_t)stream, dtype, *d);
+}
+int uia_mona_cls_bwd(void* stream, int dtype, int B, int ntok, const void* dd, const void* t, int64_t ldt, void* dt, float p_drop, uint64_t seed, const uint8_t* keep_mask) {
+    return uia_mona_cls_bwd_launch((hipStream_t)stream, dtype, B, ntok, dd, t, (long)ldt, dt, p_drop, seed, keep_mask);
+}
+int uia_copy_rows(void* stream, int rows, int64_t row_bytes, const void* src, int64_t src_stride_bytes, void* dst) {
+    return uia_copy_rows_launch((hipStream_t)stream, rows, (long)row_bytes, src, (long)src_stride_bytes, dst);
+}
 int uia_cast(void* stream, int dtype, size_t n, const float* src, void* dst, float scale) { return uia_cast_launch((hipStream_t)stream, dtype, n, src, dst, scale); }
 int uia_transpose_cast(void* stream, int dtype, int rows, int cols, const float* src, void* dst) { return uia_transpose_cast_launch((hipStream_t)stream, dtype, rows, cols, src, dst); }
 int uia_pack_weights(void* stream, int dtype, int n, const uia_pack_desc* descs_device, int max_elems) { return uia_pack_weights_launch((hipStream_t)stream, dtype, n, descs_device, max_elems); }
diff --git a/nextgen-uia_amd/csrc/cls_grad.hip b/nextgen-uia_amd/csrc/cls_grad.hip
--- /dev/null
+++ b/nextgen-uia_amd/csrc/cls_grad.hip
@@ -0,0 +1,157 @@
+#include "uia_common.h"
+#include "uia_kernels.h"
+
+namespace {
+
+__device__ __forceinline__ float sum8(float v) {
+    v += uia_dpp_quad_xor1(v);
+    v += uia_dpp_quad_xor2(v);
+    v += uia_dpp_half_mirror(v);
+    return v;
+}
+
+constexpr int ACL_THREADS = 256, ACL_KEYS = ACL_THREADS / 8;
+
+template <typename T, bool KB>
+__global__ __launch_bounds__(ACL_THREADS) void attn_bwd_cls_kernel(const UiaAttnParams p) {
+    __shared__ float red[ACL_KEYS][64];
+    const int tid = threadIdx.x, s = tid & 7, g = tid >> 3;
+    const int b = blockIdx.x / p.H, h = blockIdx.x - b * p.H, L = p.L;
+    const size_t row0 = (size_t)b * L;
+    const int col = h * 64 + 8 * s;
+    float q[8], o[8], dO[8];
+    load8((const T*)p.q + row0 * p.ld_qkv + col, q);
+    load8((const T*)p.dout + (size_t)b * p.lddo + col, dO);
+    if (KB && p.out_kb_rows) load8((const T*)p.out + ((size_t)(col >> 5) * (size_t)p.out_kb_rows + row0) * 32 + (col & 31), o);
+    else load8((const T*)p.out + row0 * p.ldo + col, o);
+    const float lse = p.lse[((size_t)b * p.H + h) * L];
+    float dl = 0.f;
+#pragma unroll
+    for (int e = 0; e < 8; ++e) dl = fmaf(dO[e], o[e], dl);
+    const float delta = sum8(dl);
+    float dq[8];
+#pragma unroll
+    for (int e = 0; e < 8; ++e) dq[e] = 0.f;
+    const float zero[8] = {0.f, 0.f, 0.f, 0.f, 0.f, 0.f, 0.f, 0.f};
+    for (int j = g; j < L; j += ACL_KEYS) {
+        const size_t row = row0 + j;
+        float k[8], v[8];
+        load8((const T*)p.k + row * p.ld_qkv + col, k);
+        load8((const T*)p.v + row * p.ld_qkv + col, v);
+        float sc = 0.f, dp = 0.f;
+#pragma unroll
+        for (int e = 0; e < 8; ++e) {
+            sc = fmaf(q[e], k[e], sc);
+            dp = fmaf(dO[e], v[e], dp);
+        }
+        sc = sum8(sc);
+        dp = sum8(dp);
+        const float P = __expf(fmaf(sc, p.scale, -lse));
+        const float dS = P * (dp - delta) * p.scale;
+        float dk[8], dv[8];
+#pragma unroll
+        for (int e = 0; e < 8; ++e) {
+            dk[e] = dS * q[e];
+            dv[e] = P * dO[e];
+            dq[e] = fmaf(dS, k[e], dq[e]);
+        }
+        if (KB && p.dqkv_kb_rows) {
+            const size_t off = ((size_t)(col >> 5) * (size_t)p.dqkv_kb_rows + row) * 32 + (col & 31);
+            store8((T*)p.dk + off, dk);
+            store8((T*)p.dv + off, dv);
+            if (j > 0) store8((T*)p.dq + off, zero);
+        } else {
+            const size_t off = row * p.ld_dqkv + col;
+            store8((T*)p.dk + off, dk);
+            store8((T*)p.dv + off, dv);
+            if (j > 0) store8((T*)p.dq + off, zero);
+        }
+    }
+#pragma unroll
+    for (int e = 0; e < 8; ++e) red[g][8 * s + e] = dq[e];
+    __syncthreads();
+    if (tid < 8) {
+        float acc[8];
+#pragma unroll
+        for (int e = 0; e < 8; ++e) acc[e] = 0.f;
+        for (int r = 0; r < ACL_KEYS; ++r)
+#pragma unroll
+            for (int e = 0; e < 8; ++e) acc[e] += red[r][8 * tid + e];
+        const int c0 = h * 64 + 8 * tid;
+        if (KB && p.dqkv_kb_rows) store8((T*)p.dq + ((size_t)(c0 >> 5) * (size_t)p.dqkv_kb_rows + row0) * 32 + (c0 & 31), acc);
+        else store8((T*)p.dq + row0 * p.ld_dqkv + c0, acc);
+    }
+}
+
+template <typename T>
+__global__ __launch_bounds__(256) void mona_cls_bwd_kernel(int B, int ntok, const T* __restrict__ dd, const T* __restrict__ t, long ldt, T* __restrict__ dt,
+                                                           float p_drop, uint64_t seed, const uint8_t* __restrict__ keep_mask) {
+    const int i = blockIdx.x * 256 + threadIdx.x;
+    if (i >= B * 64) return;
+    const int b = i >> 6, c = i & 63;
+    const float inv_keep = p_drop > 0.f ? 1.0f / (1.0f - p_drop) : 1.0f;
+    const uint32_t thresh = p_drop > 0.f ? (uint32_t)fminf(p_drop * 4294967296.0f, 4294967295.0f) : 0u;
+    const size_t idx = (size_t)b * ntok * 64 + c;
+    float ks = 1.0f;
+    if (keep_mask) ks = keep_mask[idx] ? inv_keep : 0.f;
+    else if (p_drop > 0.f) ks = dropout_keep(seed, (uint32_t)idx, thresh) ? inv_keep : 0.f;
+    const float z = to_f32(t[(size_t)b * ldt + c]);
+    dt[i] = from_f32<T>(to_f32(dd[i]) * ks * dgelu_erf(z));
+}
+
+__global__ __launch_bounds__(256) void copy_rows_kernel(int rows, int units, const uint4* __restrict__ src, long src_stride_units, uint4* __restrict__ dst) {
+    const long i = (long)blockIdx.x * 256 + threadIdx.x;
+    if (i >= (long)rows * units) return;
+    const long r = i / units, u = i - r * units;
+    dst[i] = src[r * src_stride_units + u];
+}
+
+}
+
+int uia_attn_bwd_cls_launch(hipStream_t stream, int dtype, const UiaAttnParams& p) {
+    UIA_CHECK_ARG(dtype == UIA_BF16 || dtype == UIA_F32, "uia_attn_bwd_cls: bad dtype %d", dtype);
+    UIA_CHECK_ARG(p.B > 0 && p.H > 0 && p.L > 0 && p.L <= 288, "uia_attn_bwd_cls: B=%d H=%d L=%d outside the supported range (L <= 288)", p.B, p.H, p.L);
+    UIA_CHECK_ARG(p.dh == 64, "uia_attn_bwd_cls: head dim %d, only 64 is supported", p.dh);
+    UIA_CHECK_ARG(p.mask_kind == UIA_MASK_NONE && !p.keylen && !p.cu_seqlens, "uia_attn_bwd_cls: no mask, no key lengths, no packed sequences (mask kind %d)", p.mask_kind);
+    UIA_CHECK_ARG(p.scale > 0.f && p.scale < 3.0e38f, "uia_attn_bwd_cls: scale must be positive and finite, got %g", (double)p.scale);
+    UIA_CHECK_ARG(p.q && p.k && p.v && p.out && p.dout && p.lse && p.dq && p.dk && p.dv, "uia_attn_bwd_cls: null tensor");
+    UIA_CHECK_ARG((p.out_kb_rows == 0 && p.dqkv_kb_rows == 0) ||
+                  (dtype == UIA_BF16 && (p.out_kb_rows == 0 || p.out_kb_rows >= (int64_t)p.B * p.L) && (p.dqkv_kb_rows == 0 || p.dqkv_kb_rows >= (int64_t)p.B * p.L)),
+                  "uia_attn_bwd_cls: K-blocked out / dq, dk, dv need bf16 and at least B*L rows");
+    const int esz = dtype == UIA_BF16 ? 2 : 4;
+    const int64_t width = (int64_t)p.H * 64;
+    UIA_CHECK_ARG(p.ld_qkv >= width && p.lddo >= width && (p.out_kb_rows || p.ldo >= width) && (p.dqkv_kb_rows || p.ld_dqkv >= width), "uia_attn_bwd_cls: leading dimension below H*64");
+    UIA_CHECK_ARG((p.ld_qkv * esz) % 16 == 0 && (p.ldo * esz) % 16 == 0 && (p.lddo * esz) % 16 == 0 && (p.ld_dqkv * esz) % 16 == 0,
+                  "uia_attn_bwd_cls: leading dimensions must keep 16-byte rows");
+    UIA_CHECK_ARG(((uintptr_t)p.q | (uintptr_t)p.k | (uintptr_t)p.v | (uintptr_t)p.out | (uintptr_t)p.dout | (uintptr_t)p.dq | (uintptr_t)p.dk | (uintptr_t)p.dv) % 16 == 0,
+                  "uia_attn_bwd_cls: alignment");
+    const dim3 grid(p.B * p.H), block(ACL_THREADS);
+    if (dtype == UIA_BF16) hipLaunchKernelGGL((attn_bwd_cls_kernel<bf16_t, true>), grid, block, 0, stream, p);
+    else hipLaunchKernelGGL((attn_bwd_cls_kernel<float, false>), grid, block, 0, stream, p);
+    UIA_CHECK_LAUNCH();
+    return 0;
+}
+
+int uia_mona_cls_bwd_launch(hipStream_t stream, int dtype, int B, int ntok, const void* dd, const void* t, long ldt, void* dt, float p_drop, uint64_t seed,
+                            const uint8_t* keep_mask) {
+    UIA_CHECK_ARG(dtype == UIA_BF16 || dtype == UIA_F32, "uia_mona_cls_bwd: bad dtype %d", dtype);
+    UIA_CHECK_ARG(B > 0 && ntok > 0 && (size_t)B * ntok * 64 <= 0xFFFFFFFFull, "uia_mona_cls_bwd: B=%d images of %d tokens outside the 32-bit mask index", B, ntok);
+    UIA_CHECK_ARG(dd && t && dt && ldt >= 64, "uia_mona_cls_bwd: null tensor or row stride below 64");
+    UIA_CHECK_ARG(p_drop >= 0.f && p_drop < 1.f, "uia_mona_cls_bwd: p_drop=%f outside [0, 1)", (double)p_drop);
+    const dim3 grid((B * 64 + 255) / 256), block(256);
+    if (dtype == UIA_BF16) hipLaunchKernelGGL(mona_cls_bwd_kernel<bf16_t>, grid, block, 0, stream, B, ntok, (const bf16_t*)dd, (const bf16_t*)t, ldt, (bf16_t*)dt, p_drop, seed, keep_mask);
+    else hipLaunchKernelGGL(mona_cls_bwd_kernel<float>, grid, block, 0, stream, B, ntok, (const float*)dd, (const float*)t, ldt, (float*)dt, p_drop, seed, keep_mask);
+    UIA_CHECK_LAUNCH();
+    return 0;
+}
+
+int uia_copy_rows_launch(hipStream_t stream, int rows, long row_bytes, const void* src, long src_stride_bytes, void* dst) {
+    UIA_CHECK_ARG(rows > 0 && row_bytes > 0 && row_bytes % 16 == 0 && src_stride_bytes % 16 == 0 && src_stride_bytes >= row_bytes && row_bytes / 16 <= 0x7FFFFFFF,
+                  "uia_copy_rows: %d rows of %ld bytes, %ld apart: rows and their stride must be whole 16-byte units", rows, row_bytes, src_stride_bytes);
+    UIA_CHECK_ARG(src && dst && ((uintptr_t)src | (uintptr_t)dst) % 16 == 0, "uia_copy_rows: null or misaligned tensor");
+    const int units = (int)(row_bytes / 16);
+    const long total = (long)rows * units;
+    hipLaunchKernelGGL(copy_rows_kernel, dim3((unsigned)((total + 255) / 256)), dim3(256), 0, stream, rows, units, (const uint4*)src, src_stride_bytes / 16, (uint4*)dst);
+    UIA_CHECK_LAUNCH();
+    return 0;
+}
diff --git a/nextgen-uia_amd/csrc/layernorm.hip b/nextgen-uia_amd/csrc/layernorm.hip
--- a/nextgen-uia_amd/csrc/layernorm.hip
+++ b/nextgen-uia_amd/csrc/layernorm.hip
@@ -47,12 +47,13 @@
     }
 }
 
-template <typename T, bool THREE, int NV>
+template <typename T, bool THREE, int NV, bool PERIODIC = false>
 __global__ __launch_bounds__(256, NV == 4 ? (THREE ? 3 : 5) : 1) void ln_bwd_kernel(int M, int D, long ldx, const T* __restrict__ dy, const float* __restrict__ x,
                                                       const float* __restrict__ gamma, float eps, const float* __restrict__ dres,
                                                       float* __restrict__ dx32, T* __restrict__ dxT,
                                                       const bf16_t* __restrict__ x_hi, const int8_t* __restrict__ x_lo, long x_kb_rows,
-                                                      const bf16_t* __restrict__ dres_hi, const int8_t* __restrict__ dres_lo, long dres_kb_rows, int8_t* __restrict__ dx_lo) {
+                                                      const bf16_t* __restrict__ dres_hi, const int8_t* __restrict__ dres_lo, long dres_kb_rows, int8_t* __restrict__ dx_lo,
+                                                      int period) {
     const int row = blockIdx.x * 4 + (threadIdx.x >> 6), lane = threadIdx.x & 63;
     if (row >= M) return;
     const int nv = D >> 2;
@@ -61,7 +62,7 @@
     f32x4 v[NV], g[NV];
     uint2 rhi[THREE ? NV : 1];
     unsigned rlo[THREE ? NV : 1];
-    const bool r3 = THREE && dres_lo != nullptr;
+    const bool r3 = THREE && !PERIODIC && dres_lo != nullptr;
     float s = 0.f;
 #pragma unroll
     for (int k = 0; k < NV; ++k) {
@@ -116,7 +117,9 @@
         const int c = lane + 64 * k;
         if (c < nv) {
             f32x4 o = f32x4{0.f, 0.f, 0.f, 0.f};
-            if constexpr (THREE) {
+            if constexpr (PERIODIC) {
+                if (row % period == 0) o = load4(dres + (size_t)(row / period) * D + 4 * c);
+            } else if constexpr (THREE) {
                 if (r3) o = three_byte_decode4(rhi[k], rlo[k]);
                 else if (dres) o = load4(dres + (size_t)row * ldx + 4 * c);
             } else {
@@ -173,7 +176,7 @@
     const dim3 grid((M + 3) / 4), block(256);
 #define UIA_LN_BWD(TT, TH, NVV)                                                                                                              \
     hipLaunchKernelGGL((ln_bwd_kernel<TT, TH, NVV>), grid, block, 0, stream, M, D, ldx, (const TT*)dy, x, gamma, eps, dres, dx32, (TT*)dxT,          \
-                       (const bf16_t*)x_hi, x_lo, x_kb_rows, (const bf16_t*)dres_hi, dres_lo, dres_kb_rows, dx_lo)
+                       (const bf16_t*)x_hi, x_lo, x_kb_rows, (const bf16_t*)dres_hi, dres_lo, dres_kb_rows, dx_lo, 0)
     const bool narrow = D <= 768;
     if (dtype == UIA_BF16 && three) { if (narrow) UIA_LN_BWD(bf16_t, true, 3); else UIA_LN_BWD(bf16_t, true, 4); }
     else if (dtype == UIA_BF16) { if (narrow) UIA_LN_BWD(bf16_t, false, 3); else UIA_LN_BWD(bf16_t, false, 4); }
@@ -183,3 +186,29 @@
     UIA_CHECK_LAUNCH();
     return 0;
 }
+
+int uia_layernorm_bwd_periodic_launch(hipStream_t stream, int dtype, int M, int D, const void* dy, const float* x, const void* x_hi, const int8_t* x_lo, long x_kb_rows,
+                                      const float* gamma, float eps, const float* dres_rows, int period, float* dx32, void* dxT, int8_t* dx_lo) {
+    UIA_CHECK_ARG(M > 0 && D > 0 && D % 4 == 0 && D <= 1024 && period > 0, "uia_layernorm_bwd_periodic: unsupported shape M=%d D=%d period=%d", M, D, period);
+    UIA_CHECK_ARG(dy && (x || (x_hi && x_lo)) && gamma && dres_rows && (dx32 || dxT), "uia_layernorm_bwd_periodic: null tensor");
+    UIA_CHECK_ARG(((uintptr_t)dres_rows % 16) == 0, "uia_layernorm_bwd_periodic: dres_rows must be 16-byte aligned");
+    UIA_CHECK_ARG(dtype == UIA_BF16 || dtype == UIA_F32, "uia_layernorm_bwd_periodic: bad dtype %d", dtype);
+    if (dtype == UIA_BF16)
+        UIA_CHECK_ARG(dx_lo && dxT && ((uintptr_t)dxT % 8) == 0 && ((uintptr_t)dx_lo % 4) == 0, "uia_layernorm_bwd_periodic: the bf16 form writes a three-byte result (dxT + dx_lo)");
+    else
+        UIA_CHECK_ARG(!dx_lo && !x_lo && !x_hi, "uia_layernorm_bwd_periodic: three-byte tensors need bf16");
+    UIA_CHECK_ARG(!x_lo || (x_hi && !x && (x_kb_rows == 0 || (x_kb_rows >= M && D % 32 == 0)) && ((uintptr_t)x_hi % 8) == 0 && ((uintptr_t)x_lo % 4) == 0),
+                  "uia_layernorm_bwd_periodic: x as a three-byte tensor needs x_hi + x_lo (and no fp32 x), a K-blocked hi plane of at least M rows and D a multiple of 32");
+    UIA_CHECK_ARG(x_lo || x_kb_rows == 0, "uia_layernorm_bwd_periodic: x_kb_rows without a three-byte x");
+    const dim3 grid((M + 3) / 4), block(256);
+    const long ldx = D;
+#define UIA_LN_BWD_P(TT, TH, NVV)                                                                                                                    \
+    hipLaunchKernelGGL((ln_bwd_kernel<TT, TH, NVV, true>), grid, block, 0, stream, M, D, ldx, (const TT*)dy, x, gamma, eps, dres_rows, dx32, (TT*)dxT, \
+                       (const bf16_t*)x_hi, x_lo, x_kb_rows, (const bf16_t*)nullptr, (const int8_t*)nullptr, 0L, dx_lo, period)
+    const bool narrow = D <= 768;
+    if (dtype == UIA_BF16) { if (narrow) UIA_LN_BWD_P(bf16_t, true, 3); else UIA_LN_BWD_P(bf16_t, true, 4); }
+    else { if (narrow) UIA_LN_BWD_P(float, false, 3); else UIA_LN_BWD_P(float, false, 4); }
+#undef UIA_LN_BWD_P
+    UIA_CHECK_LAUNCH();
+    return 0;
+}
diff --git a/nextgen-uia_amd/csrc/uia_kernels.h b/nextgen-uia_amd/csrc/uia_kernels.h
--- a/nextgen-uia_amd/csrc/uia_kernels.h
+++ b/nextgen-uia_amd/csrc/uia_kernels.h
@@ -19,6 +19,12 @@
 int uia_layernorm_bwd3_launch(hipStream_t stream, int dtype, int M, int D, long ldx, const void* dy, const float* x, const void* x_hi, const int8_t* x_lo,
                               long x_kb_rows, const float* gamma, float eps, const float* dres, const void* dres_hi, const int8_t* dres_lo, long dres_kb_rows,
                               float* dx32, void* dxT, int8_t* dx_lo);
+int uia_layernorm_bwd_periodic_launch(hipStream_t stream, int dtype, int M, int D, const void* dy, const float* x, const void* x_hi, const int8_t* x_lo, long x_kb_rows,
+                                      const float* gamma, float eps, const float* dres_rows, int period, float* dx32, void* dxT, int8_t* dx_lo);
+int uia_attn_bwd_cls_launch(hipStream_t stream, int dtype, const UiaAttnParams& p);
+int uia_mona_cls_bwd_launch(hipStream_t stream, int dtype, int B, int ntok, const void* dd, const void* t, long ldt, void* dt, float p_drop, uint64_t seed,
+                            const uint8_t* keep_mask);
+int uia_copy_rows_launch(hipStream_t stream, int rows, long row_bytes, const void* src, long src_stride_bytes, void* dst);
 int uia_lora_rank_update_launch(hipStream_t stream, int dtype, const uia_lora_rank_desc& p);
 int uia_ln_lora_down_launch(hipStream_t stream, int dtype, const uia_ln_lora_desc& p);
 int uia_cast_launch(hipStream_t stream, int dtype, size_t n, const float* src, void* dst, float scale);
diff --git a/nextgen-uia_amd/uia_hip/_lib.py b/nextgen-uia_amd/uia_hip/_lib.py
--- a/nextgen-uia_amd/uia_hip/_lib.py
+++ b/nextgen-uia_amd/uia_hip/_lib.py
@@ -176,6 +176,10 @@
     "uia_embed_bwd": (C.c_int, [vp, C.c_int, C.c_int, C.c_int, vp, vp, vp, C.c_int64]),
     "uia_embed_packed": (C.c_int, [vp, C.c_int, C.c_int, C.c_int, C.c_int, vp, vp, vp, vp, vp, vp]),
     "uia_gather_rows": (C.c_int, [vp, C.c_int, C.c_int, vp, vp, vp]),
+    "uia_copy_rows": (C.c_int, [vp, C.c_int, i64, vp, i64, vp]),
+    "uia_attn_bwd_cls": (C.c_int, [vp, C.c_int, C.POINTER(AttnDesc)]),
+    "uia_mona_cls_bwd": (C.c_int, [vp, C.c_int, C.c_int, C.c_int, vp, vp, i64, vp, f32, C.c_uint64, vp]),
+    "uia_layernorm_bwd_periodic": (C.c_int, [vp, C.c_int, C.c_int, C.c_int, vp, vp, vp, vp, i64, vp, f32, vp, C.c_int, vp, vp, vp]),
 }
 
 _lib = None
diff --git a/nextgen-uia_amd/uia_hip/functional.py b/nextgen-uia_amd/uia_hip/functional.py
--- a/nextgen-uia_amd/uia_hip/functional.py
+++ b/nextgen-uia_amd/uia_hip/functional.py
@@ -8,8 +8,8 @@
 
 from . import handoff, ops
 from ._lib import UiaError
-from .handoff import (Resid3, _g3_partner_feeds, fwd3_of, grad3_decode, grad3_of, grad_resid3_enabled, hook_free, linear_chain,
-                      publish_fwd3, publish_grad3, publish_rows, publish_t_copy, set_grad_resid3, t_copy_of, take_rows, zero_sums)
+from .handoff import (ClsGrad, Resid3, _g3_partner_feeds, cls_grad_of, fwd3_of, grad3_decode, grad3_of, grad_resid3_enabled, hook_free, linear_chain,
+                      publish_cls_grad, publish_fwd3, publish_grad3, publish_rows, publish_t_copy, set_cls_grad, set_grad_resid3, t_copy_of, take_rows, zero_sums)
 from .handoff import clear as clear_t_copies
 
 _STATE = {"dtype": torch.bfloat16, "seed": 0x5EED, "calls": 0, "fwd_resid3": os.environ.get("UIA_FWD_RESID3", "1") != "0"}
@@ -410,10 +410,51 @@
         ctx.meta = (variant, hw, p_drop, seed, names, keep_mask is not None)
         ctx.direct_params = tuple(params) if direct else None
         ctx.g3_out = dt == torch.bfloat16 and _g3_partner_feeds(x)
+        front = handoff.partner_node(x)
+        ctx.cls_ok = u is not None and type(front).__name__ == "VitBlockFnBackward" and handoff.takes_cls_grad(x)
         return y
 
     @staticmethod
+    def backward_cls(ctx, cg):
+        variant, hw, p_drop, seed, names, has_mask = ctx.meta
+        x, u, t, d, keep_mask, *params = ctx.saved_tensors
+        keep_mask = keep_mask if has_mask else None
+        P = dict(zip(names, params))
+        B, N, D = x.shape
+        dt, bott = u.dtype, t.shape[1]
+        dy = cg.rows32
+        dy_t = dy if dt == torch.float32 else (cg.rows_t if cg.rows_t is not None else t_copy_of(dy, dt))
+        direct = ctx.direct_params is not None and all(_is_flat_grad(p) for p in ctx.direct_params)
+        G = ({k: p.grad for k, p in zip(names, ctx.direct_params)} if direct
+             else {k: torch.zeros_like(v, dtype=torch.float32) for k, v in P.items()})
+        cls_rows = lambda a: a.view(B, N * a.shape[1])[:, :a.shape[1]]
+        side = _wgrad_side_stream(x.device) if _STATE.get("wgrad_side_stream", False) else None
+        w2t = WEIGHTS.get(P["project2.weight"], dt, transpose=True)
+        dd = _empty((B, bott), dt, x)
+        _wgrad_beside(side, lambda: ops.gemm(dy_t, w2t, out_t=dd), dy_t, cls_rows(d), G["project2.weight"], G["project2.bias"])
+        dtt = _empty((B, bott), dt, x)
+        ops.mona_cls_bwd(B, N, dd, t, dtt, p_drop=p_drop, seed=seed, keep_mask=keep_mask)
+        w1t = WEIGHTS.get(P["project1.weight"], dt, transpose=True)
+        fuse_du = x.is_cuda and ops.mona_pre_bwd_du_ok(B, D, bott, dt)
+        du = None if fuse_du else _empty((B, D), dt, x)
+        _wgrad_beside(side, None if fuse_du else (lambda: ops.gemm(dtt, w1t, out_t=du)), dtt, cls_rows(u), G["project1.weight"], G["project1.bias"])
+        need_dx = ctx.needs_input_grad[0]
+        x_cls = ops.copy_rows(x.view(B * N, D), N, _empty((B, D), torch.float32, x))
+        dx = _empty((B, D), torch.float32, x) if need_dx else None
+        dx_t = _empty((B, D), dt, x) if (need_dx and dt != torch.float32) else None
+        w1t_rows = (dtt, w1t.row if isinstance(w1t, ops.PackedW) else w1t) if fuse_du else None
+        ops.mona_pre_bwd(du, x_cls, dy if need_dx else None, P["norm.weight"], P["norm.bias"], P["gamma"], P["gammax"], dx, dx_t,
+                         G["gamma"], G["gammax"], G["norm.weight"], G["norm.bias"], dt_w1t=w1t_rows)
+        if need_dx:
+            dx = publish_cls_grad(x.shape, x.device, dx, dx_t) if ctx.cls_ok else ClsGrad(dx, dx_t, N).decode()
+        grads = tuple(None if direct else (G[k] if ctx.needs_input_grad[7 + i] else None) for i, k in enumerate(names))
+        return (dx, None, None, None, None, None, None) + grads
+
+    @staticmethod
     def backward(ctx, dy):
+        cg = cls_grad_of(dy)
+        if cg is not None:
+            return MonaFn.backward_cls(ctx, cg)
         variant, hw, p_drop, seed, names, has_mask = ctx.meta
         x, u, t, d, keep_mask, *params = ctx.saved_tensors
         keep_mask = keep_mask if has_mask else None
@@ -601,10 +642,60 @@
             ctx.xshape = (B, N, D)
             ctx.spec = spec
             ctx.g3_out = dt == torch.bfloat16 and _g3_partner_feeds(x)
+            ctx.cls_ok = spec.mask is None and N <= ATTN_SINGLE_PASS_MAX and D == 64 * spec.heads and not r3 and handoff.cls_grad_enabled()
         return x2
 
     @staticmethod
+    def backward_cls(ctx, cg):
+        xin, qkv, a, lse, x1, pre = handoff.restore_layout(ctx.saved_tensors, ctx.layout)
+        x3_in = isinstance(xin, Resid3)
+        x = xin.lo if x3_in else xin
+        spec = ctx.spec
+        B, N, D = ctx.xshape
+        M, dt = B * N, qkv.dtype
+        F = pre.shape[1]
+        dy = cg.rows32
+        dy_t = dy if dt == torch.float32 else (cg.rows_t if cg.rows_t is not None else t_copy_of(dy, dt))
+        pre_cls = ops.copy_rows(pre, N, _empty((B, F), dt, x))
+        dpre = _empty((B, F), dt, x)
+        ops.gemm(dy_t, WEIGHTS.get(spec.fc2[0], dt, transpose=True), dact=spec.act, aux_in=pre_cls, out_t=dpre)
+        dh = _empty((B, D), dt, x)
+        ops.gemm(dpre, WEIGHTS.get(spec.fc1[0], dt, transpose=True), out_t=dh)
+        x1_cls = ops.copy_rows(x1, N, _empty((B, D), torch.float32, x))
+        dx1 = _empty((B, D), torch.float32, x)
+        dx1_t = _empty((B, D), dt, x) if dt != torch.float32 else dx1
+        ops.layernorm_bwd(dh, x1_cls, spec.ln2[0], spec.eps, dres=dy, dx32=dx1, dx_t=dx1_t if dt != torch.float32 else None)
+        da = dh
+        ops.gemm(dx1_t, WEIGHTS.get(spec.proj[0], dt, transpose=True), out_t=da)
+        dqkv = _attn_act(M, 3 * D, dt, x, D)
+        if ops.is_kb(dqkv):
+            ops.attn_bwd_cls(qkv[:, :D], qkv[:, D:2 * D], qkv[:, 2 * D:], a, da, lse, dqkv, None, None, B, spec.heads, N)
+        else:
+            ops.attn_bwd_cls(qkv[:, :D], qkv[:, D:2 * D], qkv[:, 2 * D:], a, da, lse, dqkv[:, :D], dqkv[:, D:2 * D], dqkv[:, 2 * D:], B, spec.heads, N)
+        dh1 = _empty((M, D), dt, x)
+        ops.gemm(dqkv, WEIGHTS.get(spec.qkv[0], dt, transpose=True), out_t=dh1)
+        xrows = xin if x3_in else x.view(M, D)
+        if getattr(ctx, "g3_out", False):
+            dx_t = _empty((M, D), dt, x)
+            dlo = torch.empty(M, D, device=x.device, dtype=torch.int8)
+            ops.layernorm_bwd_periodic(dh1, xrows, spec.ln1[0], spec.eps, dx1, N, dx_t=dx_t, dx_lo=dlo)
+            return publish_grad3((B, N, D), x.device, dx_t, dlo), None
+        dx = torch.empty(B, N, D, device=x.device, dtype=torch.float32)
+        if dt == torch.float32:
+            ops.layernorm_bwd_periodic(dh1, xrows, spec.ln1[0], spec.eps, dx1, N, dx32=dx.view(M, D))
+            return dx, None
+        dx_t = _empty((M, D), dt, x)
+        ops.layernorm_bwd(dh1, xrows, spec.ln1[0], spec.eps, dres=ClsGrad(dx1, None, N).decode().view(M, D), dx32=dx.view(M, D), dx_t=dx_t)
+        publish_t_copy(dx, dx_t)
+        return dx, None
+
+    @staticmethod
     def backward(ctx, dx2):
+        cg = cls_grad_of(dx2)
+        if cg is not None:
+            if getattr(ctx, "cls_ok", False):
+                return VitBlockFn.backward_cls(ctx, cg)
+            dx2 = cg.decode()
         g3 = grad3_of(dx2)
         xin, qkv, a, lse, x1, pre = handoff.restore_layout(ctx.saved_tensors, ctx.layout)
         x3_in, r3 = isinstance(xin, Resid3), isinstance(x1, Resid3)
@@ -808,6 +899,7 @@
         ops.gemm(h, WEIGHTS.get(w, dt, transpose=w_is_in_out), out32=feat)
         ctx.save_for_backward(x, ln_w)
         ctx.meta = (eps, w, w_is_in_out, dt)
+        ctx.cls_out = handoff.takes_cls_grad(x, in_chain=False)
         return feat
 
     @staticmethod
@@ -832,6 +924,12 @@
             dh_t = _empty((B, D), dt, x)
             ops.cast(dh, dh_t)
             dh = dh_t
+        if getattr(ctx, "cls_out", False):
+            x_cls = ops.copy_rows(x.view(B * N, D), N, _empty((B, D), torch.float32, x))
+            rows32 = _empty((B, D), torch.float32, x)
+            rows_t = _empty((B, D), dt, x) if dt != torch.float32 else None
+            ops.layernorm_bwd(dh, x_cls, ln_w, eps, dx32=rows32, dx_t=rows_t)
+            return publish_cls_grad(x.shape, x.device, rows32, rows_t), None, None, None, None, None
         dx = torch.zeros_like(x)
         dx_t = torch.zeros(B * N, D, device=x.device, dtype=dt) if dt != torch.float32 else None
         ops.layernorm_bwd(dh, x, ln_w, eps, dx32=dx, dx_t=dx_t, rows=B, ldx=N * D)
diff --git a/nextgen-uia_amd/uia_hip/handoff.py b/nextgen-uia_amd/uia_hip/handoff.py
--- a/nextgen-uia_amd/uia_hip/handoff.py
+++ b/nextgen-uia_amd/uia_hip/handoff.py
@@ -4,7 +4,7 @@
 
 from . import ops
 
-_STATE = {"chain_depth": 0, "fwd3_next_plain": False, "grad_resid3": False}
+_STATE = {"chain_depth": 0, "fwd3_next_plain": False, "grad_resid3": False, "cls_grad": True}
 
 
 class Resid3(NamedTuple):
@@ -23,6 +23,18 @@
     @property
     def resid3(self):
         return Resid3(self.hi, self.lo)
+
+
+class ClsGrad(NamedTuple):
+    rows32: torch.Tensor
+    rows_t: object
+    tokens: int
+
+    def decode(self):
+        B, D = self.rows32.shape
+        dense = self.rows32.new_zeros(B, self.tokens, D)
+        dense[:, 0] = self.rows32
+        return dense
 
 
 def save_layout(*values):
@@ -78,6 +90,7 @@
 
 GRAD3 = TokenRegistry(64)
 FWD3 = TokenRegistry(256)
+CLSG = TokenRegistry(64)
 _G3_VIEWS = ("PermuteBackward0", "ViewBackward0", "UnsafeViewBackward0", "TransposeBackward0", "AliasBackward0", "ReshapeAliasBackward0")
 _G3_PARTNERS = ("MonaFnBackward", "VitBlockFnBackward")
 
@@ -100,6 +113,22 @@
 
 def fwd3_of(x):
     return FWD3.take(x)
+
+
+def publish_cls_grad(shape, device, rows32, rows_t):
+    return CLSG.publish(shape, device, ClsGrad(rows32, rows_t, shape[1]))
+
+
+def cls_grad_of(g):
+    return CLSG.take(g)
+
+
+def set_cls_grad(flag):
+    _STATE["cls_grad"] = bool(flag)
+
+
+def cls_grad_enabled():
+    return _STATE["cls_grad"] and _STATE["grad_resid3"]
 
 
 def set_grad_resid3(flag):
@@ -142,20 +171,28 @@
     return True
 
 
-def _g3_partner_feeds(x):
-    if not _STATE["grad_resid3"] or _STATE["chain_depth"] <= 0:
-        return False
+def partner_node(x, in_chain=True):
+    if not _STATE["grad_resid3"] or (in_chain and _STATE["chain_depth"] <= 0):
+        return None
     fn = x.grad_fn
     for _ in range(8):
         if fn is None:
-            return False
+            return None
         name = type(fn).__name__
         if name in _G3_PARTNERS:
-            return True
+            return fn
         if name not in _G3_VIEWS or len(fn.next_functions) != 1:
-            return False
+            return None
         fn = fn.next_functions[0][0]
-    return False
+    return None
+
+
+def _g3_partner_feeds(x):
+    return partner_node(x) is not None
+
+
+def takes_cls_grad(x, in_chain=True):
+    return cls_grad_enabled() and bool(getattr(partner_node(x, in_chain), "cls_ok", False))
 
 
 _T_COPIES = {}
@@ -218,3 +255,4 @@
     _SUMS_ARENA.clear()
     GRAD3.clear()
     FWD3.clear()
+    CLSG.clear()
diff --git a/nextgen-uia_amd/uia_hip/ops.py b/nextgen-uia_amd/uia_hip/ops.py
--- a/nextgen-uia_amd/uia_hip/ops.py
+++ b/nextgen-uia_amd/uia_hip/ops.py
@@ -824,6 +824,31 @@
         check(lib().uia_attn_bwd(_stream(), _code(q.dtype), C.byref(d)), "uia_attn_bwd")
 
 
+def attn_bwd_cls(q, k, v, out, dout, lse, dq, dk, dv, B, H, L, mask=None, scale=None):
+    if mask not in (None, "none"):
+        raise UiaError(f"attn_bwd_cls: mask {mask!r}: the CLS-query backward takes unmasked attention only")
+    d = _attn_desc(q, k, v, out, lse, B, H, L, None, None, scale)
+    if d.dh != 64:
+        raise UiaError(f"attn_bwd_cls: head dim {d.dh}, only 64 is supported")
+    if dout.dim() != 2 or dout.shape[0] != B or dout.shape[1] != H * 64 or dout.stride(1) != 1 or dout.dtype != q.dtype:
+        raise UiaError(f"attn_bwd_cls: dout must be [{B}, {H * 64}] {q.dtype} rows (one per sequence), got {tuple(dout.shape)} {dout.dtype}")
+    if lse is None or lse.dtype != torch.float32 or not lse.is_contiguous() or lse.numel() != B * H * L:
+        raise UiaError(f"attn_bwd_cls: lse must be a contiguous fp32 [{B}, {H}, {L}] tensor")
+    d.dout, d.lddo = _p(dout), dout.stride(0)
+    if is_kb(dq):
+        rows, cols, d.dqkv_kb_rows = _kb_dims(dq, "attention dqkv")
+        if rows < B * L or cols != 3 * H * 64 or q.dtype != torch.bfloat16 or dk is not None or dv is not None:
+            raise UiaError(f"attention dqkv (K-blocked {tuple(dq.t.shape)}) must hold [{B * L}, {3 * H * 64}] bf16 with head dim 64, dk = dv = None")
+        part = (H * 64 // kb_group(q.dtype)) * d.dqkv_kb_rows * kb_group(q.dtype) * dq.t.element_size()
+        d.dq, d.dk, d.dv, d.ld_dqkv = dq.t.data_ptr(), dq.t.data_ptr() + part, dq.t.data_ptr() + 2 * part, cols
+    else:
+        for name, t in (("dq", dq), ("dk", dk), ("dv", dv)):
+            if t.dtype != q.dtype or t.dim() != 2 or t.shape[0] < B * L or t.shape[1] != H * 64 or t.stride(1) != 1 or t.stride(0) != dq.stride(0):
+                raise UiaError(f"attn_bwd_cls: {name} must be [{B * L}, {H * 64}] {q.dtype} rows sharing one row stride, got {tuple(t.shape)} {t.dtype}")
+        d.dq, d.dk, d.dv, d.ld_dqkv = _p(dq), _p(dk), _p(dv), dq.stride(0)
+    check(lib().uia_attn_bwd_cls(_stream(), _code(q.dtype), C.byref(d)), "uia_attn_bwd_cls")
+
+
 def layernorm_fwd(x, gamma, beta, eps, y_t=None, y32=None, rows=None, ldx=None, stats=None):
     D = gamma.numel()
     rows = x.numel() // D if rows is None else rows
@@ -878,6 +903,26 @@
                                        None if isinstance(dres, tuple) else _p(dres), _p(r_hi), _p(r_lo), r_kb, _p(dx32), _p(dx_t), _p(dx_lo)), "uia_layernorm_bwd3")
         return
     check(lib().uia_layernorm_bwd(_stream(), _code(dy.dtype), rows, D, ldx, _p(dy), _p(x), _p(gamma), eps, _p(dres), _p(dx32), _p(dx_t)), "uia_layernorm_bwd")
+
+
+def layernorm_bwd_periodic(dy, x, gamma, eps, dres_rows, period, dx32=None, dx_t=None, dx_lo=None):
+    D = gamma.numel()
+    M = dy.numel() // D
+    nrows = (M + period - 1) // period
+    _dense(dres_rows, "layernorm_bwd_periodic: dres_rows", _F32, nrows * D, align=16)
+    x_hi, x_lo = x if isinstance(x, tuple) else (None, None)
+    x_kb = 0
+    if is_kb(x_hi):
+        kr, kc, x_kb = _kb_dims(x_hi, "layernorm_bwd_periodic x hi plane")
+        if kr < M or kc != D:
+            raise UiaError(f"layernorm_bwd_periodic: K-blocked x hi plane {tuple(x_hi.t.shape)} does not hold [{M}, {D}]")
+        x_hi = x_hi.t
+    for name, t, dt_ in (("dy", dy, dy.dtype), ("x", None if isinstance(x, tuple) else x, torch.float32), ("x hi", x_hi, torch.bfloat16), ("x lo", x_lo, torch.int8),
+                         ("dx32", dx32, torch.float32), ("dx_t", dx_t, dy.dtype), ("dx_lo", dx_lo, torch.int8)):
+        if t is not None and (t.dtype != dt_ or not t.is_contiguous() or t.numel() < M * D):
+            raise UiaError(f"layernorm_bwd_periodic: {name} must be a contiguous {dt_} tensor of at least [{M}, {D}], got {tuple(t.shape)} {t.dtype}")
+    check(lib().uia_layernorm_bwd_periodic(_stream(), _code(dy.dtype), M, D, _p(dy), None if isinstance(x, tuple) else _p(x), _p(x_hi), _p(x_lo), x_kb, _p(gamma), eps,
+                                           _p(dres_rows), int(period), _p(dx32), _p(dx_t), _p(dx_lo)), "uia_layernorm_bwd_periodic")
 
 
 def cast(src, dst, scale=1.0):
@@ -1015,6 +1060,16 @@
     check(lib().uia_gather_rows(_stream(), idx.numel(), src.shape[-1], _p(src), _p(idx), _p(dst)), "uia_gather_rows")
 
 
+def copy_rows(src, stride_rows, dst):
+    if src.dim() != 2 or dst.dim() != 2 or not src.is_contiguous() or not dst.is_contiguous() or src.dtype != dst.dtype or src.shape[1] != dst.shape[1]:
+        raise UiaError(f"copy_rows: contiguous 2-D tensors of one dtype and width are required, got {tuple(src.shape)} {src.dtype} -> {tuple(dst.shape)} {dst.dtype}")
+    rows, row_bytes = dst.shape[0], src.shape[1] * src.element_size()
+    _require(rows > 0 and stride_rows > 0 and (rows - 1) * stride_rows < src.shape[0], f"copy_rows: {rows} rows {stride_rows} apart do not fit the {src.shape[0]} rows of src")
+    _require(row_bytes % 16 == 0 and src.data_ptr() % 16 == 0 and dst.data_ptr() % 16 == 0, "copy_rows: rows must be whole, aligned 16-byte units")
+    check(lib().uia_copy_rows(_stream(), rows, row_bytes, _p(src), row_bytes * stride_rows, _p(dst)), "uia_copy_rows")
+    return dst
+
+
 _SPATIAL_KEYS = ("conv1_w", "conv1_b", "conv2_w", "conv2_b", "conv3_w", "conv3_b", "proj_w", "proj_b", "freq", "ne1_w", "ne1_b", "ne3_w", "ne3_b")
 
 
@@ -1143,6 +1198,15 @@
     check(lib().uia_mona_spatial_bwd(_stream(), _code(t.dtype), C.byref(d)), "uia_mona_spatial_bwd")
 
 
+def mona_cls_bwd(B, ntok, dd, t, dt, p_drop=0.0, seed=0, keep_mask=None):
+    for name, x_, n in (("dd", dd, B * 64), ("dt", dt, B * 64), ("t", t, B * ntok * 64)):
+        _dense(x_, f"mona_cls_bwd: {name}", (t.dtype,), n, align=2)
+    if keep_mask is not None:
+        _dense(keep_mask, "mona_cls_bwd: keep_mask", (torch.uint8,), B * ntok * 64)
+    check(lib().uia_mona_cls_bwd(_stream(), _code(t.dtype), B, ntok, _p(dd), _p(t), ntok * 64, _p(dt), float(p_drop), int(seed) & 0xFFFFFFFFFFFFFFFF, _p(keep_mask)),
+          "uia_mona_cls_bwd")
+
+
 def infonce(img, txt, temperature, grad_scale=1.0, want_grads=True):
     assert img.dtype == torch.float32 and txt.dtype == torch.float32 and img.is_contiguous() and txt.is_contiguous()
     B, E = img.shape
```

New measurement: 6642, median of 6. 2.3% higher.
